# ishovkun/poroelasticity-dealii

Measured on AMD Instinct MI355X. Metric: DoF-updates/sec in assemble+SpMV per fixed-stress iter, higher is better.
Workload: dtype f64

## Files before the change

poroelasticity_dealii_amd/csrc/common.hpp:

```cpp
#pragma once
#include <hip/hip_runtime.h>
#include <cstdint>
#include <cstdio>
#include <map>
#include <memory>
#include <type_traits>
#include <stdexcept>
#include <string>
#include <list>
#include <vector>
#include "../../include/poroel_hip.h"
#include "fdm_tables.hpp"
#include "cell_field.hpp"

namespace poro {

#define PORO_HIP(x)                                                                                   \
  do { hipError_t e_ = (x); if (e_ != hipSuccess) throw poro::Error(std::string(#x) + " -> " + hipGetErrorString(e_)); } while (0)

template <class T> struct DevBuf {
  T *p = nullptr; size_t n = 0;
  DevBuf() = default; DevBuf(const DevBuf &) = delete; DevBuf &operator=(const DevBuf &) = delete;
  ~DevBuf() { release(); }
  void release() { if (p) (void)hipFree(p); p = nullptr; n = 0; }
  void alloc(size_t n_) { release(); n = n_; if (n) PORO_HIP(hipMalloc((void **)&p, n * sizeof(T))); }
  void zero(hipStream_t s) { if (n) PORO_HIP(hipMemsetAsync(p, 0, n * sizeof(T), s)); }
  void upload(const T *h, size_t n_) { alloc(n_); if (n) PORO_HIP(hipMemcpy(p, h, n * sizeof(T), hipMemcpyHostToDevice)); }
  void upload(const std::vector<T> &h) { upload(h.data(), h.size()); }
};

constexpr int kMaxPartials = 1024;
constexpr int kScalarSlots = 32;

struct PcgScalars {
  double dh, gg, gz;
  double gh2[2];
  double alpha, beta;
  double tol, res0, res;
  int32_t it, done, converged, max_iter, finishing;
  int32_t stop;
};
struct PcgStopTest { PcgScalars *sc = nullptr; const double *gg_part = nullptr; int it = 0; int per_wave = 0; };
static_assert(sizeof(PcgStopTest) == 24, "PcgStopTest is embedded in kernel arguments");

struct Mailbox { volatile unsigned long long seq; unsigned long long pad_; double vals[16]; PcgScalars sc; };

struct Cg1State { double gamma_old, alpha_old, alpha, beta, tol, res0, res; int32_t it, done, converged, pad_; };

struct DiagVec { const double *full = nullptr; const uint8_t *cls = nullptr; const double *tab = nullptr; int ncomp = 1; };

struct FeTablesDev {
  int nq_u, nq_p, nq_f, ns_u, ns_p;
  const double *w_qu, *w_qp, *w_qf, *u_qu, *du_qu, *du_qp, *q1_qu, *dq1_qu, *q1_qp, *dq1_qp, *u_qf, *dq1_qf;
};

struct BoxCoupling { int k; int n[3]; double h[3]; double N[3][2], D[3][2]; };

struct FdmDir { int n = 0; DevBuf<double> S, St, lam; };
struct FdmScalar { int dim = 0; FdmDir dir[3]; bool built = false; };
struct FdmScale { const double *lam[3]; int n[3]; double a, k[3]; int64_t ncol, col0, col_total; };
struct FdmWindow { int n_planes; int64_t ncols_valid, grid_col0, grid_plane0; };
struct SlabLayout {
  int n_ranks = 1, rank = 0;
  std::vector<int> layers, off;
  int ng = 0;
  int64_t ncol_total = 0, C = 0;
  int max_own = 0, max_nl = 0;
};
struct FdmDist : SlabLayout {
  bool built = false;
  FdmDir last;
  DevBuf<double> sendbuf, recvbuf, tz1, tz2; std::vector<double> hsend, hrecv;
  DevBuf<FdmWindow> windows;
};

struct FdmuDir { int n = 0; bool reg_form = false, split = false, blk = false; int n_even = 0; int blk_kk[2] = {0, 0}, blk_nch[2] = {0, 0}, blk_mb[2] = {0, 0} ; DevBuf<double> fwd, bwd, lam; };
struct FdmU : SlabLayout {
              int dim = 0; int nn[3] = {1, 1, 1}; double coef[3][3] = {}; FdmuDir dir[3][3]; FdmuDir last_global[3]; bool built = false, single = false;
              int fix[3][3][2] = {};
              bool dist = false; DevBuf<double> sendbuf, recvbuf, tz1, tz2;
              bool line = false; DevBuf<double> line_coef, line_fac; };
struct FdmoPlans;
constexpr double kFdmoStripFill = 0.4;
struct FdmOct {
  bool built = false; int nt = 0;
  int n[3] = {1, 1, 1}, h[3] = {1, 1, 1}; int hxp = 2;
  int64_t co_stride = 0, n_oct = 0;
  double coef[3][3] = {};
  DevBuf<double> fwd[3][3][2], bwd[3][3][2], lam[3][3][2];
  DevBuf<float> fwd32[3][3][2], bwd32[3][3][2];
  DevBuf<double> g, z, t;
  DevBuf<double> gz_part; int gz_n = 0;
  std::vector<double> h_lam[3][3][2];
  DevBuf<double> bxy;
  int no = 8;
  int nc = 3;
  bool planar = false;
  int own_z = 0;
  bool per_dir = false; int split_mask = 7, nt_z = 0;
  struct Slab {
    bool on = false; int n_ranks = 1, rank = 0;
    int ng = 0, hzg = 0;
    bool zboth = false; DevBuf<int64_t> dst2;
    int np = 2, nb = 12;
    int cw = 64, nchunk = 0, cps = 0, chunk0 = 0, my_chunks = 0;
    int64_t scols = 0;
    int own = 0, nl = 0, max_own = 0, max_nl = 0, rows_back = 0;
    int64_t recv_off = 0;
    DevBuf<int64_t> row_in;
    DevBuf<int64_t> row_out; DevBuf<int32_t> row_kz;
    DevBuf<double> buf, tz;
  } slab;
  std::shared_ptr<FdmoPlans> plans;
  struct ScalarTable { double a, kappa; DevBuf<double> t; };
  std::list<ScalarTable> scalar_tables;
  double strip_limit = 0;
};
struct FdmQ1 { FdmScalar nodal; FdmOct fused; };
struct SsorLevels { DevBuf<int32_t> fwd_rows, bwd_rows; std::vector<int64_t> fwd_off, bwd_off; bool built = false; };
struct CsrDev {
  int64_t n = 0, nnz = 0;
  DevBuf<int64_t> rp; DevBuf<int32_t> col; DevBuf<int64_t> diag_pos;
  int lanes_per_row = 8;
  SsorLevels ssor;
};

struct ConsDev {
  int64_t n = 0, n_masters = 0;
  DevBuf<int32_t> dof, master; DevBuf<int64_t> ptr; DevBuf<double> weight, inhom;
  DevBuf<int32_t> t_master, t_dof; DevBuf<int64_t> t_ptr; DevBuf<double> t_weight;
  DevBuf<uint8_t> inert;
  DevBuf<uint8_t> hanging;
  bool any_inhom = false;
};

struct Timer { double seconds = 0; int64_t launches = 0 , enqueued = 0 ; std::vector<std::pair<hipEvent_t, hipEvent_t>> pending;
               bool sample(int stride) { return enqueued++ % stride == 0; } };

struct IfcDev {
  int64_t m_send = 0, m_shared = 0, n_owned = 0;
  std::vector<int64_t> ptr;
  DevBuf<int32_t> dof, sh_dof, sh_src; DevBuf<int64_t> sh_ptr; DevBuf<double> send, recv;
  std::vector<double> hsend, hrecv;
};

struct Comm {
  poro_partition part{};
  bool general = false; std::vector<int32_t> neighbours; IfcDev ifc_u, ifc_p;
  void *nccl_comm = nullptr;
  poro_allreduce_fn ar = nullptr; poro_sendrecv_fn sr = nullptr; void *user = nullptr;
  DevBuf<double> recv_lo, recv_hi; std::vector<double> hsend, hrecv;
  struct Pinned { double *p = nullptr; size_t n = 0; Pinned() = default; Pinned(const Pinned &) = delete; Pinned &operator=(const Pinned &) = delete; ~Pinned() { if (p) (void)hipHostFree(p); } } hvec;
  bool force_multi = false;
  bool multi() const { return part.n_ranks > 1 || force_multi; }
};

struct KellyDev { bool built = false; int64_t n_faces = 0; DevBuf<int32_t> cell_a, cell_b, code, ent_face, ent_hcell; DevBuf<int64_t> ent_ptr; DevBuf<double> jump, eta; };

struct HybridPlan {
  bool built = false;
  int64_t n_box_nodes = 0, n_fine_cells = 0, n_removed = 0, n_chunks = 0;
  DevBuf<int64_t> inj;
  DevBuf<int32_t> color_cells; std::vector<int64_t> color_off;
  DevBuf<int32_t> spatial_cells;
  DevBuf<int32_t> removed_cells, slot;
  DevBuf<uint8_t> touched;
  DevBuf<double> Ke_t, V;
  DevBuf<int64_t> nodes; DevBuf<int32_t> chunk_cls;
  DevBuf<double> x_box, y_box;
};

struct BoxDev { int enabled = 0; int n[3] = {1, 1, 1}; int nn[3] = {1, 1, 1}; double h[3] = {1, 1, 1}; };

}

struct poro_ctx {
  poro_ctx() = default; poro_ctx(const poro_ctx &) = delete; poro_ctx &operator=(const poro_ctx &) = delete;
  ~poro_ctx() { if (mailbox) (void)hipHostFree(mailbox); }
  int device = 0, operator_mode = PORO_OP_CSR;
  hipStream_t stream = nullptr;
  int dim = 2, k_u = 2, ns_u = 9, ns_p = 4, dpc_u = 18, dpc_p = 4, nv = 4;
  int64_t n_cells = 0, n_u = 0, n_p = 0;
  poro_material mat{};
  poro::BoxDev box;
  struct Lines { bool on = false, uniform = true; int n[3] = {1, 1, 1}, nn[3] = {1, 1, 1}; std::vector<double> hcell[3]; } lines;
  poro::Comm comm;
  poro::DevBuf<int32_t> cell_dofs_u, cell_dofs_p, color_cells;
  poro::DevBuf<double> cell_X, tables;
  poro::DevBuf<double> cell_geo;
  poro::FeTablesDev fe{};
  int mfg_sf = 0;
  std::vector<int64_t> color_off;
  int scatter_mode = 0; poro::DevBuf<int32_t> spatial_cells;
  int operator_form = 0; poro::HybridPlan hyb;
  int fdm_precision = 0;
  int fdm_form = 0; bool fdm_form_fixed = false;
  poro::DevBuf<uint8_t> dir_mask, node_mask; poro::DevBuf<double> dir_val; poro::DevBuf<int32_t> dir_dofs;
  std::vector<int32_t> h_dir_dof; std::vector<double> h_dir_val;
  poro::ConsDev cons_u, cons_p;
  poro::DevBuf<uint8_t> pdir_mask; poro::DevBuf<double> pdir_val; int64_t n_pdir = 0;
  bool pdir_faces_ok = false; int pdir_face[3][2] = {{0, 0}, {0, 0}, {0, 0}};
  poro::DevBuf<int32_t> bface_cell, bface_local, bface_id, neu_label, neu_comp; poro::DevBuf<double> neu_val;
  poro::DevBuf<int32_t> bface_order; std::vector<int64_t> bface_group_off;
  int64_t n_bfaces = 0; int n_neumann = 0;
  poro::CsrDev Ap, Au;
  poro::DevBuf<double> Mp, Kp, Jp, Au_val;
  bool projection_matrix_ready = false;
  poro::DevBuf<double> Ke;
  std::map<int, poro::DevBuf<double>> vec, vec_saved;
  poro::DevBuf<uint8_t> rhs_u_flags;
  poro::DevBuf<double> lift_u, neumann_u, diag_u, diag_u_local, diag_J, diag_M, src_local;
  poro::DevBuf<double> dinv_u, dinv_J, dinv_M;
  poro::DevBuf<uint8_t> diag_u_cls; poro::DevBuf<double> diag_u_tab;
  poro::DevBuf<double> wg_u, wd_u, wh_u, wg_p, wd_p, wh_p, tmp_p, proj_y;
  bool box_asm_checked = false;
  int box_asm = 0 ; poro::BoxCoupling box_cpl{};
  poro::DevBuf<double> ilu_u, ilu_J, ilu_M; bool ilu_u_valid = false, ilu_J_valid = false, ilu_M_valid = false;
  poro::DevBuf<double> wz_p;
  poro::FdmQ1 q1_free, q1_fixed; poro::FdmDist fdm_dist; poro::DevBuf<double> fdm_t1, fdm_t2;
  double cheb_lmax = 0;
  double cheb_ratio_default = 0;
  poro::DevBuf<double> cheb_z, cheb_t;
  poro::FdmOct fdm_oct;
  struct Interp { int64_t n_fine = 0, n_coarse = 0; int lanes = 1, lanes_t = 1;    poro::DevBuf<int64_t> p_ptr, pt_ptr; poro::DevBuf<int32_t> p_col, pt_col; poro::DevBuf<double> p_w, pt_w; };
  struct TwoLevel : Interp { poro_ctx *box = nullptr; Interp pressure; bool pdir_nested = false;  } two_level;
  bool borrowed_stream = false;
  poro::FdmU fdm_u; poro::DevBuf<double> fdmu_t1, fdmu_t2, wz_u; int fdm_u_state = 0 ; std::string fdm_u_why;
  std::vector<uint8_t> h_node_mask;
  poro::DevBuf<double> partials; poro::DevBuf<poro::PcgScalars> scal; poro::DevBuf<double> red;
  poro::Mailbox *mailbox = nullptr; unsigned long long mb_seq = 0;
  int timing_stride = 1;
  poro::DevBuf<double> cheb_side_lo, cheb_side_hi;
  poro::DevBuf<poro::Cg1State> cg1_state; poro::DevBuf<double> cg1_z[2], cg1_w[2];
  bool matrix_built = false;
  int interleaved_u = 0;
  int pcg_hint_fdm_u[2] = {0, 0}, pcg_hint_cheb_u[2] = {0, 0}; int64_t cheb_applies = 0;
  int pcg_hint_u[2] = {0, 0};
  int pcg_hint_p[2] = {0, 0}, pcg_hint_proj[2] = {0, 0};
  int n_cus = 256; int mf_variant = 1 ; int mask_anywhere = 0;
  bool timing = false; std::map<std::string, poro::Timer> timers; std::vector<hipEvent_t> event_pool;
  double jac_dt = -1;
  poro::KellyDev kelly;
  struct Perm : poro::CellField<3> {
    int ncomp = 0;
    poro::DevBuf<double> cell, lattice;
    struct Line { bool built = false; int lo = 0, hi = 0; double a = -1; poro::DevBuf<double> coef, inv; } line[2];
  } perm;
  struct Moduli : poro::CellField<2> { poro::DevBuf<double> cell, node, planes; } mod;
  int moduli_op = 0;
  struct Gravity {
    bool on = false, loads_stale = false; double g[3] = {0, 0, 0}, rho_b = 0, rho_f = 0;
    struct Density : poro::CellField<1> { poro::DevBuf<double> cell, lattice; } dens;
    poro::DevBuf<double> body_u, flux_p, src_p;
    bool flux_on() const { return on && rho_f != 0; }
  } grav;
};

namespace poro {

inline bool box_fast_u(const poro_ctx *c) { return c->box.enabled && !c->mod.kind; }
inline bool moduli_structured_applies(const poro_ctx *c) {
  return c->box.enabled && c->dim == 3 && (c->k_u == 1 || c->k_u == 2) && c->mod.kind == 1 && c->operator_mode == PORO_OP_MATRIX_FREE && c->mf_variant == 1 && !c->comm.multi() &&
         c->comm.part.n_ranks <= 1;
}
inline bool moduli_structured(const poro_ctx *c) { return c->moduli_op == PORO_MODULI_OP_STRUCTURED && c->mod.planes.p && moduli_structured_applies(c); }

void la_fill(hipStream_t s, double *x, double v, int64_t n);
void la_nodal_interp(hipStream_t s, const int64_t *ptr, const int32_t *col, const double *w, int64_t n_rows, int ncomp, const double *in, double *out, int lanes = 1);
void la_two_level_combine(hipStream_t s, const int64_t *ptr, const int32_t *col, const double *w, int64_t n_rows, int ncomp, const double *zc, const double *g, const double *dinv, const uint8_t *inert, double omega, double *z, int lanes = 1);
void la_copy_many(hipStream_t s, int count, double *const *dst, const double *const *src, const int64_t *n);
void la_post(hipStream_t s, Mailbox *mb, unsigned long long seq, const double *src, int n, const PcgScalars *sc);
void la_reduce_post(hipStream_t s, const double *partials, int n_sets, double *red, int max_not_sum_mask, Mailbox *mb, unsigned long long seq);
void la_copy(hipStream_t s, double *y, const double *x, int64_t n);
void la_axpy(hipStream_t s, double *y, double a, const double *x, int64_t n);
void la_add_range(hipStream_t s, double *y, const double *x, int64_t n);
void la_add_two_ranges(hipStream_t s, double *y0, const double *x0, double *y1, const double *x1, int64_t n);
void la_dot_partials(hipStream_t s, const double *a, const double *b, int64_t n, double *partials , const PcgScalars *gate = nullptr );
void la_norm_partials(hipStream_t s, const double *a, int64_t n, double *partials_l2, double *partials_inf);
void la_reduce_finish(hipStream_t s, const double *partials, int n_sets, double *red , int max_not_sum_mask);
void la_csr_spmv(hipStream_t s, const CsrDev &A, const double *val, const double *x, double *y);
void la_csr_residual(hipStream_t s, const CsrDev &A, const double *M, const double *K, double kappa, const double *t, const double *p,
                     const double *src, double *R);
void la_pressure_tmp(hipStream_t s, double *t, const double *ev, const double *ev0, const double *p, const double *p_old, double c1, double c2, int64_t n);
void la_jacobian(hipStream_t s, double *J, const double *M, const double *K, double a, double kappa, int64_t nnz);
void la_ifc_pack(hipStream_t s, const IfcDev &I, const double *v);
void la_ifc_sum(hipStream_t s, const IfcDev &I, double *v);
void la_csr_diag(hipStream_t s, const CsrDev &A, const double *val, double *diag);
void la_reciprocal(hipStream_t s, double *y, const double *x, int64_t n);
void la_pointwise_mul(hipStream_t s, double *y, const double *x, int64_t n);
void la_cheb_first(hipStream_t s, double *z, const double *g, const DiagVec &dv, double scale, int64_t n);
void la_cheb_step(hipStream_t s, double *znew, const double *zj, const double *g, const double *Az, const DiagVec &dv, double omega, int64_t n, int64_t n_owned, double *gz_partials);
void la_cheb_fix_planes(hipStream_t s, double *znew, const double *zj, const double *g, const double *own_lo, const double *nbr_lo, const double *own_hi, const double *nbr_hi, const DiagVec &dv, double omega, int64_t n, int64_t plane);
void la_cons_expand(hipStream_t s, const ConsDev &C, double *x, bool with_inhom);
void la_cons_reduce(hipStream_t s, const ConsDev &C, double *y);
void la_xpby(hipStream_t s, double *y, double a, double b, const double *x, int64_t n);
void la_ilu0_factor(hipStream_t s, const CsrDev &A, const SsorLevels &lv, double *lu , int *flag );
void la_ilu_apply(hipStream_t s, const CsrDev &A, const double *lu, const SsorLevels &lv, const double *src, double *dst);
void la_ssor_apply(hipStream_t s, const CsrDev &A, const double *val, const SsorLevels &lv, double omega, const double *src, double *dst);
void la_sum_strains(hipStream_t s, double *ev, const double *const *strains, int n, int64_t len);
void la_effective_stress(hipStream_t s, const double *const *strains, double *const *stresses, int dim, double lam, double G, int64_t len);
void la_effective_stress_nodal(hipStream_t s, const double *const *strains, double *const *stresses, int dim, const double *node_mod, int64_t len);
void la_strain_update_nodal(hipStream_t s, double *ev, const double *dp, double alpha, const double *node_mod, int64_t len);
void la_set_constrained(hipStream_t s, double *x, const uint8_t *mask, const double *val, int64_t n);
void la_rhs_u_finish(hipStream_t s, double *rhs, const double *lift, const double *neumann, const uint8_t *mask, int64_t n);
void pcg_init_residual(hipStream_t s, double *g, const double *Ax, const double *b, const uint8_t *inert , int64_t n);
void la_mask_zero(hipStream_t s, double *x, const uint8_t *mask, int64_t n);
void pcg_dot_dh(hipStream_t s, const PcgScalars *sc, const double *d, const double *h, int64_t n_owned, double *partials);
void pcg_first_direction(hipStream_t s, double *d, const double *g, const DiagVec &diag, const double *z, int prec, int64_t n, int64_t n_owned, double *partials );
void pcg_scalars_sum(hipStream_t s, const double *partials, int n_sets, double *red);
void cg1_dots(hipStream_t s, const double *g, const double *z, const double *w, const double *b , int64_t n_owned, double *partials );
void cg1_scalars(hipStream_t s, Cg1State *st, const double *red, int first, double abs_tol, double rel_tol, int max_iter, int stop_rule);
void cg1_update(hipStream_t s, const Cg1State *st, double *d, double *sv, double *x, double *g, const double *z, const double *w, const DiagVec &dv, const uint8_t *inert,
                double *z1_out , double z1_scale, int64_t n);
void pcg_scalars_start(hipStream_t s, PcgScalars *sc, const double *red , double abs_tol, double rel_tol, int max_iter, int stop_rule);
void pcg_update_g_fused(hipStream_t s, PcgScalars *sc, int parity, double *g, const double *h, const DiagVec &diag, const double *z, double *z1_out , double z1_scale, int prec, int64_t n, int64_t n_owned,
                        const double *partials_dh, const double *red , double *partials_out );
void pcg_update_d_fused(hipStream_t s, PcgScalars *sc, int parity, int it, double *x, double *d, const double *g, const DiagVec &diag, const double *z, int prec, int64_t n,
                        const double *partials_in , const double *red );

void kelly_faces(hipStream_t s, int dim, int64_t n_faces, const int32_t *cell_a, const int32_t *cell_b, const int32_t *code, const double *cell_X, const int32_t *cell_dofs_p,
                 const double *p, double *jump);
void kelly_cells(hipStream_t s, int dim, int64_t n_cells, const int64_t *ent_ptr, const int32_t *ent_face, const int32_t *ent_hcell, const double *cell_X, const double *jump, double *eta);
void transfer_rows3(hipStream_t s, int64_t n_rows, const int64_t *ptr, const int32_t *col, const double *w, const double *const in[3], double *const out[3]);

struct AsmArgs {
  int dim, k_u, ns_u, ns_p, nv, dpc_u;
  FeTablesDev fe;
  const int32_t *cell_dofs_u, *cell_dofs_p; const double *cell_X;
  const double *cell_geo;
  const uint8_t *dir_mask; const double *dir_val;
  poro_material mat;
  int interleaved_u;
  int mfg_sf;
  const double *cell_mod;
};
void asm_u_matrix(hipStream_t s, const AsmArgs &a, const int32_t *cells, int64_t n_cells, const int64_t *rp, const int32_t *col, double *val, double *lift);
void asm_u_element_matrix(hipStream_t s, const AsmArgs &a, int32_t cell, double *Ke);
void asm_u_rhs(hipStream_t s, const AsmArgs &a, const int32_t *cells, int64_t n_cells, const double *p, double *rhs);
void asm_u_neumann(hipStream_t s, const AsmArgs &a, const int32_t *order, const std::vector<int64_t> &group_off, const int32_t *bf_cell, const int32_t *bf_local, const int32_t *bf_id,
                   int n_neu, const int32_t *label, const int32_t *comp, const double *value, double *rhs);
void asm_p_matrices(hipStream_t s, const AsmArgs &a, const int32_t *cells, int64_t n_cells, const int64_t *rp, const int32_t *col, double *M, double *K, double *src, const double *cell_w = nullptr,
                    int ncomp = 1);
void asm_proj_rhs(hipStream_t s, const AsmArgs &a, const int32_t *cells, int64_t n_cells, const double *u, int n_comp, const int32_t *comps ,
                  double *const *rhs );

void box_body_u(hipStream_t s, int dim, int k_u, const BoxDev &box, const double *rho_lattice, double rho0, const double *g, double *out);
void box_gravity_p(hipStream_t s, int dim, const BoxDev &box, const double *kap_lattice, int ncomp, double kap0, double rho_f, const double *g, double *out);
void asm_u_body(hipStream_t s, const AsmArgs &a, const int32_t *cells, int64_t n_cells, const double *cell_rho, double rho0, const double *g, double *out);
void asm_p_gravity(hipStream_t s, const AsmArgs &a, const int32_t *cells, int64_t n_cells, const double *cell_w, int ncomp, double kap0, double rho_f, const double *g, double *out);

bool mfg_sf_tables_match(const poro_fe_tables &f, int dim, int k);
int mfg_apply(hipStream_t s, const AsmArgs &a, const int32_t *color_cells, const std::vector<int64_t> &color_off, int64_t n_u, const double *x, double *y, bool constrained, int mode,
              const int32_t *all_cells = nullptr );
struct MfArgs { int dim, k_u; BoxDev box; const double *Ke; const uint8_t *mask; const double *diag_local; double lam, G; int mask_anywhere; const uint8_t *nodemask; const int32_t *dirichlet_dofs; int64_t n_dirichlet; };
void mf_apply(hipStream_t s, const MfArgs &a, const double *x, double *y, bool constrained, double *dot_partials = nullptr);
void mf_diag(hipStream_t s, const MfArgs &a, double *diag);
void p_stencil_apply(hipStream_t s, int dim, const BoxDev &box, double a, double kappa, const double *x, double *y);
void p_residual_stencil(hipStream_t s, int dim, const BoxDev &box, double kappa, const double *t, const double *p, const double *src, double *R);
void p_stencil_apply_var(hipStream_t s, int dim, const BoxDev &box, double a, const double *kap, int ncomp, const double *x, double *y);
void p_residual_stencil_var(hipStream_t s, int dim, const BoxDev &box, const double *kap, int ncomp, const double *t, const double *p, const double *src, double *R);

struct KronCheb { const double *g = nullptr; double *znew = nullptr; double omega = 0; const uint8_t *cls = nullptr; const double *tab = nullptr;
                  double *side_lo = nullptr, *side_hi = nullptr; };
bool kron_supported(int dim, int k_u);
void kron_prepare_device();
BoxCoupling box_coupling(int dim, int k_u, const BoxDev &box);
void box_rhs_u(hipStream_t s, int dim, const BoxCoupling &B, double alpha, const double *p, const double *lift, const double *neu, const uint8_t *mask, double *rhs,
               const uint8_t *flags = nullptr );
int64_t box_rhs_u_flag_count(int64_t n_u);
void box_rhs_u_flags(hipStream_t s, const double *lift, const double *neu, int64_t n_u, uint8_t *flags );
void box_asm_u_matrix(hipStream_t s, int dim, int k_u, const BoxDev &box, const double *Ke, const CsrDev &A, const uint8_t *mask, double *val);
void box_proj_rhs(hipStream_t s, int dim, const BoxCoupling &B, const double *u, int n_comp, const int32_t *tensor_components, double *const *rhs);
void fdm_window_batch(hipStream_t s, double *grid, double *dense, double *dense_self, int self, bool to_block, const FdmWindow *win, int n_peers, int n_planes_pad, int64_t C, int64_t grid_stride, int64_t blk);
void fdm_window(hipStream_t s, double *dst, const double *src, bool to_block, int n_planes, int n_planes_pad, int64_t C, int64_t ncols_valid, int64_t grid_stride, int64_t grid_col0, int64_t grid_plane0);
void fdm_transform(hipStream_t s, const double *T, int n_l, int64_t SI, int64_t n_outer, const double *in, double *out, const FdmScale *scale);
void q1_line_factor(hipStream_t s, int dim, int nw, const FdmScalar &F, int nl, double a, const double *coef, double *inv);
void q1_line_solve(hipStream_t s, int dim, int nw, const FdmScalar &F, int nl, double a, bool fixed_lo, bool fixed_hi, const double *coef, const double *inv, const double *in, double *out);
void fdm_apply(hipStream_t s, const FdmScalar &F, double a, const double k[3], const double *g, double *z, double *t1, double *t2);
void fdmu_upload_dir(FdmuDir &D, const LineTables &T, bool single, bool split);
void fdmu_apply(hipStream_t s, const FdmU &F, const double *g, double *z, void *t1, void *t2, int stage);
void fdmu_window(hipStream_t s, double *dst, const double *src, bool to_block, int ncomp, int n_planes, int n_planes_pad, int64_t C, int64_t ncols_valid,
                 int64_t grid_stride, int64_t grid_planes, int64_t grid_col0, int64_t grid_plane0);
void fdmu_lines(hipStream_t s, const FdmU &F, const FdmuDir *last_dir, int64_t C, int64_t col0, int64_t ncol_valid, void *in, void *out);
struct FdmuLineArgs { int nl, n0; int64_t ncol; const double *coef; const double *lam0[3], *lam1[3]; int fixed[3][2]; };
void fdmu_line_factor(hipStream_t s, int ku, int ncomp, const FdmuLineArgs &a, double *fac );
void fdmu_line_solve(hipStream_t s, int ku, int ncomp, const FdmuLineArgs &a, const double *fac, double *v );
bool fdmo_usable(int dim, const int nn[3]);
void fdmo_init(FdmOct &O, const int nn[3], const double coef[3][3], hipStream_t s);
void fdmo_init_slab(FdmOct &O, const int nn[3], const double coef[3][3], int rank, const std::vector<int> &node_layers, bool has_upper, hipStream_t s);
void fdmo_init_per_direction(FdmOct &O, const int nn[3], const double coef[3][3], const FdmFormDecision &D, hipStream_t s);
void fdmo_upload_dir(FdmOct &O, int comp, int dir, const LineTables &T);
void fdmo_finalize(FdmOct &O);
void fdmo_apply(hipStream_t s, const FdmOct &O, const double *g_oct, double *z_oct, double *scratch_oct, const PcgScalars *gate = nullptr, hipEvent_t *ev  = nullptr,
                double *gz_part  = nullptr,
                int precision  = PORO_FDM_FP64,
                const PcgStopTest &stop = PcgStopTest{} );
bool fdmo_scalar_usable(int dim, const int nn[3]);
void fdmo_scalar_init(FdmOct &O, const int nn[3], hipStream_t s);
void fdmo_scalar_upload_dir(FdmOct &O, int dir, const LineTables &T);
int fdmo_scalar_apply(hipStream_t s, FdmOct &O, double a, double kappa, const double *g, double *z, const PcgScalars *gate = nullptr);
int fdmo_scalar_apply_many(hipStream_t s, FdmOct &O, double a, double kappa, int nb, const double *const *g, double *const *z, const PcgScalars *gate = nullptr);
void la_residual_norms_many(hipStream_t s, int nb, const double *const *y, const double *const *b, int64_t n, double *partials, const uint8_t *mask = nullptr);
void fdmo_scalar_init_slab(FdmOct &O, const int nn[3], int rank, const std::vector<int> &node_layers, hipStream_t s);
void fdmo_scalar_slab_pass(hipStream_t s, FdmOct &O, int pass, double a, double kappa, const double *in, double *out);
bool fdmo_planar_usable(int dim, const int nn[3]);
void fdmo_init_planar(FdmOct &O, const int nn[3], const double coef[3][3], hipStream_t s, bool split = true );
void fdmo_upload_dir_planar(FdmOct &O, int comp, int dir, const LineTables &T);
void fdmo_apply_planar(hipStream_t s, const FdmOct &O, const double *g_q, double *z_q, const PcgScalars *gate = nullptr, const PcgStopTest &stop = PcgStopTest{} );
void fdmo_from_nodal(hipStream_t s, const FdmOct &O, const double *v_nodal, double *q_oct);
void fdmo_to_nodal(hipStream_t s, const FdmOct &O, const double *r_oct, double *v_nodal);
void fdmo_init_residual(hipStream_t s, const FdmOct &O, double *g_oct, const double *Ax, const double *b, const uint8_t *inert);
void fdmo_first_direction(hipStream_t s, const FdmOct &O, double *d, const double *g_oct, const double *z_oct, double *partials );
void fdmo_update_g(hipStream_t s, const FdmOct &O, PcgScalars *sc, int parity, double *g_oct, const double *h, const uint8_t *inert, const double *partials_dh, double *partials_out , const double *red = nullptr);
void fdmo_update_d(hipStream_t s, const FdmOct &O, PcgScalars *sc, int parity, int it, double *x, double *d, const double *z_oct, const double *partials_in , const double *red = nullptr,
                   bool gz_from_pass = false ,
                   bool stream_x = false ,
                   bool decided = false ,
                   bool gg_stored = false );
void fdmo_dot_owned(hipStream_t s, const FdmOct &O, const double *a_oct, const double *b_oct, double *partials, const PcgScalars *gate);
void fdmo_slab_pass(hipStream_t s, const FdmOct &O, int pass , const double *in, double *out, const PcgScalars *gate, hipEvent_t e0 = nullptr, hipEvent_t e1 = nullptr);
void fdmo_slab_scatter_pack(hipStream_t s, const FdmOct &O, const PcgScalars *gate);
int kron_apply(hipStream_t s, const MfArgs &a, const double *x, double *y, bool constrained, int n_cus, double *dot_partials = nullptr, hipEvent_t ev0 = nullptr, hipEvent_t ev1 = nullptr,
               const PcgScalars *pcg = nullptr ,
               const KronCheb *cheb = nullptr );
void kron_fix_constrained(hipStream_t s, const MfArgs &a, const double *x, double *y, double *dot_partials, int slot_base);
void kron_lm_prepare_device();
int kron_lm_apply(hipStream_t s, const MfArgs &a, const double *planes, const double *x, double *y, bool constrained, int n_cus, double *dot_partials = nullptr, hipEvent_t ev0 = nullptr,
                  hipEvent_t ev1 = nullptr, const PcgScalars *pcg = nullptr);
void hyb_gather(hipStream_t s, int dim, int64_t n_box_nodes, const int64_t *inj, const double *x, double *x_box);
struct HybCombine { int64_t n_box_nodes, n_removed, n_chunks; const int64_t *inj; const uint8_t *touched; const int32_t *removed_cells, *slot, *chunk_cls; const int64_t *nodes;
                    const double *x_box, *y_box; double *V; };
void hyb_combine(hipStream_t s, const MfArgs &box, const double *Ke_t, bool constrained, const HybCombine &h, double *y);

}
```

poroelasticity_dealii_amd/csrc/ctx_prec.hip:

```cpp
#include <dlfcn.h>
#include <rccl/rccl.h>
#include <algorithm>
#include <array>
#include <chrono>
#include <cmath>
#include <cstdlib>
#include <cstring>
#include <functional>
#include <new>
#include <optional>
#include <thread>
#include <unordered_map>
#include "common.hpp"
#include "ctx_internal.hpp"
#include "perm_line.hpp"
#include "moduli_line.hpp"

using namespace poro;
using namespace poro::ctx_detail;

namespace poro {
namespace ctx_detail {
bool fdm_p_supported(poro_ctx *c) {
  if (!c->lines.on) return false;
// ... 107 lines not shown
      PORO_HIP(hipMemcpyAsync(recv + (size_t)q * blk, F.hrecv.data(), blk * sizeof(double), hipMemcpyHostToDevice, c->stream)); PORO_HIP(hipStreamSynchronize(c->stream));
    }
  } else throw Error("partitioned context without a communicator");
}
void count_strip_launches(poro_ctx *c, int n) { if (n) c->timers["fdm_q1_strip_launches"].enqueued += n; }
void fdm_precondition_p(poro_ctx *c, double a, const double k[3], const double *g, double *z, Q1Set which) {
  Timed tm(c, "precondition_p_fdm");
  hipStream_t s = c->stream;
  const bool fixed = which == Q1Set::fixed_ends, isotropic = k[0] == k[1] && k[1] == k[2];
  FdmQ1 &T = q1_set(c, which);
  if (fixed || !c->comm.multi()) {
    std::optional<Timed> tf; if (fixed) tf.emplace(c, "precondition_p_fdm_fixed_ends");
    if (T.fused.built && isotropic) count_strip_launches(c, fdmo_scalar_apply(s, T.fused, a, k[0], g, z));
    else fdm_apply(s, T.nodal, a, k, g, z, c->fdm_t1.p, c->fdm_t2.p);
    return;
  }
  if (T.fused.built && T.fused.slab.on && isotropic) {
    FdmOct &O = T.fused; auto &S = O.slab; double *send = S.buf.p, *recv = S.buf.p + S.recv_off;
    fdmo_scalar_slab_pass(s, O, 1, a, k[0], g, S.buf.p);
    alltoall_blocks(c, send, recv, (int64_t)S.max_own * S.scols, true);
    fdmo_scalar_slab_pass(s, O, 2, a, k[0], S.buf.p, S.tz.p);
    fdmo_slab_scatter_pack(s, O, nullptr);
    alltoall_blocks(c, send, recv, (int64_t)S.max_nl * S.scols, true);
    fdmo_scalar_slab_pass(s, O, 3, a, k[0], S.buf.p, z);
    return;
  }
  FdmDist &F = c->fdm_dist; const FdmScalar &L = T.nodal;
  const int dim = c->dim, N = F.n_ranks, r = F.rank, last = dim - 1;
  const int n0 = L.dir[0].n, nl = c->box.n[last] + 1;
  const int64_t SIp = F.ncol_total;
  double *t1 = c->fdm_t1.p, *t2 = c->fdm_t2.p;
  const double *cur = g;
  if (dim == 3) { fdm_transform(s, L.dir[0].St.p, n0, 1, (int64_t)L.dir[1].n * nl, g, t1, nullptr); fdm_transform(s, L.dir[1].St.p, L.dir[1].n, n0, nl, t1, t2, nullptr); cur = t2; }
  else { fdm_transform(s, L.dir[0].St.p, n0, 1, nl, g, t1, nullptr); cur = t1; }
  const int64_t blk1 = (int64_t)F.max_own * F.C;
  fdm_window_batch(s, const_cast<double *>(cur), F.sendbuf.p, F.recvbuf.p, r, true, F.windows.p, N, F.max_own, F.C, SIp, blk1);
  alltoall_blocks(c, F.sendbuf.p, F.recvbuf.p, blk1, true);
  fdm_window_batch(s, F.tz1.p, F.recvbuf.p, nullptr, r, false, F.windows.p + N, N, F.max_own, F.C, F.C, blk1);
  FdmScale sc{}; sc.a = a; sc.ncol = F.C; sc.col0 = (int64_t)r * F.C; sc.col_total = F.ncol_total;
  for (int d = 0; d < 3; ++d) { sc.lam[d] = d < dim ? (d == last ? F.last.lam.p : L.dir[d].lam.p) : nullptr; sc.k[d] = d < dim ? k[d] : 0.0; sc.n[d] = d < dim ? (d == last ? F.ng : L.dir[d].n) : 1; }
  fdm_transform(s, F.last.St.p, F.ng, F.C, 1, F.tz1.p, F.tz2.p, &sc);
  fdm_transform(s, F.last.S.p, F.ng, F.C, 1, F.tz2.p, F.tz1.p, nullptr);
  const int64_t blk2 = (int64_t)F.max_nl * F.C;
  fdm_window_batch(s, F.tz1.p, F.sendbuf.p, F.recvbuf.p, r, true, F.windows.p + 2 * N, N, F.max_nl, F.C, F.C, blk2);
  alltoall_blocks(c, F.sendbuf.p, F.recvbuf.p, blk2, true);
  double *back = dim == 3 ? t2 : t1;
  fdm_window_batch(s, back, F.recvbuf.p, nullptr, r, false, F.windows.p + 3 * N, N, F.max_nl, F.C, SIp, blk2);
  if (dim == 3) { fdm_transform(s, L.dir[1].S.p, L.dir[1].n, n0, nl, t2, t1, nullptr); fdm_transform(s, L.dir[0].S.p, n0, 1, (int64_t)L.dir[1].n * nl, t1, z, nullptr); }
  else fdm_transform(s, L.dir[0].S.p, n0, 1, nl, t1, z, nullptr);
}

void fdm_precondition_p_layered(poro_ctx *c, double a, const double *g, double *z, Q1Set which) {
  Timed tm(c, "precondition_p_fdm_layered");
  const bool fixed = which == Q1Set::fixed_ends; const int last = c->dim - 1, nl = c->lines.n[last] + 1;
  poro_ctx::Perm &P = c->perm;
  if (!P.kind || c->comm.multi()) throw Error("fdm_precondition_p_layered: needs a per-cell permeability on a single-rank context");
  FdmQ1 &T = q1_set(c, which);
  const int nw = P.ncomp == 1 ? 1 : last;
  poro_ctx::Perm::Line &L = P.line[fixed ? 1 : 0];
  if (!L.built) {
    L.lo = fixed && c->pdir_face[last][0]; L.hi = fixed && c->pdir_face[last][1];
    L.coef.upload(perm_line_coefficients(c->lines.hcell[last], P.layer, nw, P.layer[P.ncomp - 1], L.lo, L.hi));
    if (L.inv.n != (size_t)c->n_p) L.inv.alloc(c->n_p);
    L.a = -1; L.built = true;
  }
  if (L.a != a) { q1_line_factor(c->stream, c->dim, nw, T.nodal, nl, a, L.coef.p, L.inv.p); L.a = a; }
  hipStream_t s = c->stream; const FdmScalar &F = T.nodal; const int n0 = F.dir[0].n, n1 = F.dir[1].n; double *t1 = c->fdm_t1.p, *t2 = c->fdm_t2.p;
  auto lines = [&](const double *in, double *out) { Timed tl(c, "q1_line_solve"); q1_line_solve(s, c->dim, nw, F, nl, a, L.lo, L.hi, L.coef.p, L.inv.p, in, out); };
  if (c->dim == 2) {
    fdm_transform(s, F.dir[0].St.p, n0, 1, nl, g, t1, nullptr);
    lines(t1, t2);
    fdm_transform(s, F.dir[0].S.p, n0, 1, nl, t2, z, nullptr);
  } else {
    fdm_transform(s, F.dir[0].St.p, n0, 1, (int64_t)n1 * nl, g, t1, nullptr);
    fdm_transform(s, F.dir[1].St.p, n1, n0, nl, t1, t2, nullptr);
    lines(t2, t1);
    fdm_transform(s, F.dir[1].S.p, n1, n0, nl, t1, t2, nullptr);
    fdm_transform(s, F.dir[0].S.p, n0, 1, (int64_t)n1 * nl, t2, z, nullptr);
  }
}

void analyse_fdm_u(poro_ctx *c) {
  if (c->fdm_u_state != 0) return;
  c->fdm_u_state = -1;
  const bool multi = c->comm.multi();
  if (multi && !(c->comm.nccl_comm || (c->comm.ar && c->comm.sr))) { c->fdm_u_state = 0; c->fdm_u_why = "partitioned context without a communicator yet"; return; }
  const int dim = c->dim, last = dim - 1; const int64_t nn[3] = {c->lines.nn[0], c->lines.nn[1], dim == 3 ? c->lines.nn[2] : 1};
  std::string why;
  FdmU &F = c->fdm_u;
  if (!c->lines.on || !c->interleaved_u || (multi && !c->box.enabled)) why = "needs a uniform box (or, on one rank, a tensor-product grid) with node-interleaved displacement dofs";
  else {
    for (int d = 0; d < dim; ++d) if (nn[d] > 4096) why = "more than 4096 nodes per grid line";
  }
  if (why.empty()) {
    const std::vector<uint8_t> &nm = c->h_node_mask;
    int physical[3][2] = {{1, 1}, {1, 1}, {1, 1}};
    if (multi) { physical[last][0] = !c->comm.part.has_lower; physical[last][1] = !c->comm.part.has_upper; }
    for (int comp = 0; comp < dim && why.empty(); ++comp)
      if (!whole_faces(nn, dim, nm.data(), comp, physical, F.fix[comp])) why = "Dirichlet dofs are not a union of whole faces per component";
  }
  if (multi) {
    double h[kScalarSlots] = {0}; int m = 0;
    for (int comp = 0; comp < 3; ++comp) for (int d = 0; d < 3; ++d) for (int side = 0; side < 2; ++side) h[m++] = (comp < dim && d < dim) ? F.fix[comp][d][side] : 0;
    h[m++] = why.empty() ? 0.0 : 1.0;
    PORO_HIP(hipMemcpyAsync(c->red.p, h, m * sizeof(double), hipMemcpyHostToDevice, c->stream));
    allreduce_sum(c, c->red.p, m);
    PORO_HIP(hipMemcpyAsync(h, c->red.p, m * sizeof(double), hipMemcpyDeviceToHost, c->stream)); PORO_HIP(hipStreamSynchronize(c->stream));
    m = 0;
    for (int comp = 0; comp < 3; ++comp) for (int d = 0; d < 3; ++d) for (int side = 0; side < 2; ++side) { if (comp < dim && d < dim) F.fix[comp][d][side] = h[m] > 0.5 ? 1 : 0; ++m; }
    if (h[m] > 0.5 && why.empty()) why = "another rank's Dirichlet dofs are not face-separable";
  }
  if (why.empty()) for (int d = 0; d < dim; ++d) {
    const int64_t line = (multi && d == last) ? 0 : nn[d];
    if (line > 320 && !(dim == 2 && !multi)) for (int comp = 0; comp < dim; ++comp) if (F.fix[comp][d][0] != F.fix[comp][d][1]) why = "a grid line of more than 320 points needs the same Dirichlet condition at both of its ends (even / odd transforms)";
  }
  if (why.empty()) for (int comp = 0; comp < dim; ++comp) {
    bool any = false;
    for (int d = 0; d < dim; ++d) any = any || F.fix[comp][d][0] || F.fix[comp][d][1];
    if (!any) why = "a displacement component without a constrained face (singular block)";
  }
  c->fdm_u_why = why;
  c->fdm_u_state = why.empty() ? 1 : -1;
}
void release_fdm_u(poro_ctx *c) {
  if (!c->fdm_u.built) return;
  PORO_HIP(hipStreamSynchronize(c->stream));
  c->fdm_oct.~FdmOct(); new (&c->fdm_oct) FdmOct();
  c->fdm_u.~FdmU(); new (&c->fdm_u) FdmU();
  c->fdm_u_state = 0; c->fdm_u_why.clear();
}
void build_fdm_u(poro_ctx *c) {
  FdmU &F = c->fdm_u;
  if (F.built) return;
  analyse_fdm_u(c);
  if (c->fdm_u_state != 1) throw Error("PORO_PREC_FDM (displacement): " + c->fdm_u_why);
  const int dim = c->dim, last = dim - 1, ku = c->k_u;
  const bool multi = c->comm.multi();
  const bool line = c->mod.kind != 0;
  if (line && multi) throw Error("PORO_PREC_FDM (displacement): per-cell moduli on a partitioned context");
  F.dim = dim; F.single = !multi && !line && std::getenv("PORO_FDMU_SINGLE") != nullptr;
  for (int d = 0; d < 3; ++d) F.nn[d] = d < dim ? c->lines.nn[d] : 1;
  const double l2g = c->mat.lame_lambda + 2 * c->mat.shear_G, G = c->mat.shear_G;
  for (int comp = 0; comp < dim; ++comp) for (int d = 0; d < dim; ++d) F.coef[comp][d] = d == comp ? l2g : G;
  int n_cells_last = c->lines.n[last];
  if (multi) {
    int64_t ncol_total = 1; for (int d = 0; d < last; ++d) ncol_total *= F.nn[d];
    F.dist = true; n_cells_last = slab_layout(c, F, ku, ncol_total);
    if (F.ng > 4096) throw Error("PORO_PREC_FDM (displacement): more than 4096 nodes per global grid line");
    const int N = F.n_ranks;
    const size_t blk = (size_t)dim * std::max(F.max_own, F.max_nl) * F.C;
    F.sendbuf.alloc(blk * N); F.recvbuf.alloc(blk * N); F.tz1.alloc((size_t)dim * F.ng * F.C); F.tz2.alloc((size_t)dim * F.ng * F.C);
    F.sendbuf.zero(c->stream); F.recvbuf.zero(c->stream); F.tz1.zero(c->stream); F.tz2.zero(c->stream);
  }
  LineTables tables[3][4]; bool same_ends[3], parity[3], parity_cd[3][3] = {};
  const auto key_of = [&](int comp, int d) { return F.fix[comp][d][0] * 2 + F.fix[comp][d][1]; };
  for (int d = 0; d < dim; ++d) {
    if (line && d == last) { same_ends[d] = parity[d] = false; continue; }
    const bool global_dir = multi && d == last;
    const std::vector<double> hcell = global_dir ? std::vector<double>((size_t)n_cells_last, c->box.h[d]) : c->lines.hcell[d];
    same_ends[d] = parity[d] = true;
    for (int comp = 0; comp < dim; ++comp) {
      LineTables &T = tables[d][key_of(comp, d)];
      if (!T.n) T = line_tables(ku, hcell, F.fix[comp][d][0], F.fix[comp][d][1]);
      same_ends[d] = same_ends[d] && F.fix[comp][d][0] == F.fix[comp][d][1]; parity[d] = parity[d] && T.parity; parity_cd[comp][d] = T.parity;
    }
  }
  bool oct_ok = !F.single && !line && !std::getenv("PORO_FDMU_NO_OCT");
  bool per_dir = false; FdmFormDecision form;
  bool planar = false;
  { int nn3[3] = {F.nn[0], F.nn[1], F.nn[2]}, sym3[3] = {F.nn[0], F.nn[1], multi ? F.ng : F.nn[2]};
    planar = dim == 2 && !multi && fdmo_planar_usable(dim, nn3);
    oct_ok = oct_ok && (planar || fdmo_usable(dim, sym3));
    bool symmetric = true, all_parity = true;
    for (int d = 0; d < dim; ++d) { symmetric = symmetric && same_ends[d]; all_parity = all_parity && parity[d]; }
    oct_ok = oct_ok && ((planar && !symmetric) || (symmetric && all_parity));
    if (c->fdm_form == PORO_FDM_FORM_PER_DIRECTION && !c->fdm_form_fixed && dim == 3 && !multi && !F.single && !line && !std::getenv("PORO_FDMU_NO_OCT")) {
      form = fdm_form_decide(F.fix, parity_cd, nn3);
      per_dir = form.usable && !form.all_split;
    }
    if (per_dir) { fdmo_init_per_direction(c->fdm_oct, nn3, F.coef, form, c->stream); oct_ok = true; }
    else if (oct_ok && planar) fdmo_init_planar(c->fdm_oct, nn3, F.coef, c->stream, symmetric);
    else if (oct_ok && !multi) fdmo_init(c->fdm_oct, nn3, F.coef, c->stream);
    if (oct_ok && multi) { std::vector<int> node_layers(F.n_ranks); for (int q = 0; q < F.n_ranks; ++q) node_layers[q] = ku * F.layers[q];
                           fdmo_init_slab(c->fdm_oct, nn3, F.coef, F.rank, node_layers, c->comm.part.has_upper != 0, c->stream); } }
  for (int d = 0; d < dim; ++d) for (int comp = 0; comp < dim; ++comp) {
    if (line && d == last) continue;
    const bool global_dir = multi && d == last;
    const LineTables &T = tables[d][key_of(comp, d)];
    FdmuDir &D = global_dir ? F.last_global[comp] : F.dir[comp][d];
    if (!(planar && oct_ok && T.n > 320 && !same_ends[d])) fdmu_upload_dir(D, T, global_dir ? false : F.single, same_ends[d] && parity[d]);
    if (oct_ok) { if (planar) fdmo_upload_dir_planar(c->fdm_oct, comp, d, T); else fdmo_upload_dir(c->fdm_oct, comp, d, T); }
  }
  c->fdmu_t1.alloc(c->n_u); c->fdmu_t2.alloc(c->n_u); c->fdmu_t1.zero(c->stream); c->fdmu_t2.zero(c->stream);
  if (!c->wz_u.p) { c->wz_u.alloc(c->n_u); c->wz_u.zero(c->stream); }
  if (oct_ok && !planar) fdmo_finalize(c->fdm_oct);
  c->fdm_oct.built = oct_ok;
  if (line) {
    std::vector<double> coef;
    for (int comp = 0; comp < dim; ++comp) {
      const std::vector<double> cc = moduli_line_coefficients(dim, ku, comp, c->lines.hcell[last], c->mod.layer[0], c->mod.layer[1], F.fix[comp][last][0] != 0, F.fix[comp][last][1] != 0);
      coef.insert(coef.end(), cc.begin(), cc.end());
    }
    F.line_coef.upload(coef);
    F.line_fac.alloc((size_t)(ku + 1) * c->n_u);
    F.line = true;
    fdmu_line_factor(c->stream, ku, dim, fdmu_line_args(c), F.line_fac.p);
  }
  F.built = true;
}
FdmuLineArgs fdmu_line_args(poro_ctx *c) {
  const FdmU &F = c->fdm_u; const int dim = F.dim, last = dim - 1;
  FdmuLineArgs a{};
  a.nl = F.nn[last]; a.n0 = F.nn[0]; a.ncol = c->n_u / dim / a.nl; a.coef = F.line_coef.p;
  for (int comp = 0; comp < dim; ++comp) {
    a.lam0[comp] = F.dir[comp][0].lam.p; a.lam1[comp] = dim == 3 ? F.dir[comp][1].lam.p : nullptr;
    a.fixed[comp][0] = F.fix[comp][last][0]; a.fixed[comp][1] = F.fix[comp][last][1];
  }
  return a;
}
static void fdm_precondition_u_slab(poro_ctx *c, const double *g, double *z, const PcgScalars *gate) {
  hipStream_t s = c->stream; FdmOct &O = c->fdm_oct; auto &S = O.slab;
  double *send = S.buf.p, *recv = S.buf.p + S.recv_off;
  fdmo_slab_pass(s, O, 1, g, S.buf.p, gate);
  alltoall_blocks(c, send, recv, (int64_t)S.max_own * S.scols, true);
  if (S.zboth) { Timed tp(c, "fdm_u_slab_z_stage"); fdmo_slab_pass(s, O, 2, S.buf.p, S.buf.p, gate); }
  else {
    fdmo_slab_pass(s, O, 2, S.buf.p, S.tz.p, gate);
    Timed tp(c, "fdm_u_slab_z_stage"); fdmo_slab_scatter_pack(s, O, gate);
  }
  alltoall_blocks(c, send, recv, (int64_t)S.max_nl * S.scols, true);
  fdmo_slab_pass(s, O, 3, S.buf.p, z, gate);
}
bool fdm_precondition_u_form(poro_ctx *c, const double *g, double *z, const PcgScalars *gate, int precision, double *scratch, double *gz_part, const PcgStopTest &stop) {
  Timed tm(c, "precondition_u_fdm");
  const FdmOct &O = c->fdm_oct;
  if (O.slab.on) { if (stop.gg_part) throw Error("fdm_precondition_u_form: the slab form runs no stopping test"); fdm_precondition_u_slab(c, g, z, gate); return false; }
  if (O.planar) { fdmo_apply_planar(c->stream, O, g, z, gate, stop); return false; }
  const char *names[3] = {"fdm_u_pass1", "fdm_u_pass2", "fdm_u_pass3"};
  if (!begin_sampled_dispatch(c, names[0])) {
    fdmo_apply(c->stream, O, g, z, scratch, gate, nullptr, gz_part, precision, stop);
    return gz_part != nullptr;
  }
  c->timers[names[1]].enqueued++;
  c->timers[names[2]].enqueued++;
  hipEvent_t ev[6];
  for (auto &e : ev) e = event_get(c);
  fdmo_apply(c->stream, O, g, z, scratch, gate, ev, gz_part, precision, stop);
  for (int k = 0; k < 3; ++k) {
    Timer &t = c->timers[names[k]];
    t.pending.emplace_back(ev[2 * k], ev[2 * k + 1]);
    t.launches++;
  }
  return gz_part != nullptr;
}
void fdm_precondition_u_nodal(poro_ctx *c, const double *g, double *z, int precision) {
  FdmOct &O = c->fdm_oct;
  if (!O.built) { fdm_precondition_u(c, g, z); return; }
  fdmo_from_nodal(c->stream, O, g, O.g.p); fdm_precondition_u_form(c, O.g.p, O.z.p, nullptr, precision, O.t.p); fdmo_to_nodal(c->stream, O, O.z.p, z);
}
static void upload_interp(poro_ctx::Interp &T, int64_t n_fine, int64_t n_owned, int64_t n_coarse, const int64_t *ptr, const int32_t *node, const double *weight, const char *what,
                          int row_bound = 0) {
  T.n_fine = n_fine; T.n_coarse = n_coarse;
  validate_rows(ptr, node, weight, n_fine, n_coarse, std::string("poro_desc.coarse: ") + what);
  const int64_t nnz = ptr[n_fine], nnz_t = ptr[n_owned];
  const auto lanes_for = [](int64_t nnz, int64_t rows) { return nnz >= 6 * rows ? 8 : nnz >= 3 * rows ? 4 : 1; };
  T.lanes = row_bound > 0 ? lanes_for(row_bound, 1) : lanes_for(nnz, n_fine); T.lanes_t = lanes_for(nnz_t, n_coarse);
  std::vector<int64_t> tp((size_t)n_coarse + 1, 0);
  for (int64_t k = 0; k < nnz_t; ++k) tp[node[k] + 1]++;
  { int64_t longest = 0; for (int64_t j = 0; j < n_coarse; ++j) longest = std::max(longest, tp[j + 1]);
    if (longest >= 48) T.lanes_t = std::max(T.lanes_t, 16); }
  for (int64_t j = 0; j < n_coarse; ++j) tp[j + 1] += tp[j];
  std::vector<int32_t> tc((size_t)nnz_t); std::vector<double> tw((size_t)nnz_t); std::vector<int64_t> pos(tp.begin(), tp.end() - 1);
  for (int64_t i = 0; i < n_fine; ++i) {
    if (i < n_owned) for (int64_t k = ptr[i]; k < ptr[i + 1]; ++k) { const int64_t at = pos[node[k]]++; tc[at] = (int32_t)i; tw[at] = weight[k]; }
  }
  T.p_ptr.upload(ptr, (size_t)n_fine + 1); T.p_col.upload(node, (size_t)nnz); T.p_w.upload(weight, (size_t)nnz);
  T.pt_ptr.upload(tp); T.pt_col.upload(tc); T.pt_w.upload(tw);
}
void setup_two_level(poro_ctx *c, const poro_desc *d) {
  auto &T = c->two_level; const int dim = c->dim;
  const bool general = c->comm.general;
  upload_interp(T, c->n_u / dim, general ? c->comm.ifc_u.n_owned / dim : c->n_u / dim, T.box->n_u / dim, d->coarse.ptr, d->coarse.node, d->coarse.weight, "displacement",
                general ? ipow(c->k_u + 1, dim) : 0);
  if (d->coarse.ptr_p) {
    if (!d->coarse.node_p || !d->coarse.weight_p) throw Error("poro_desc.coarse: node_p / weight_p missing");
    upload_interp(T.pressure, c->n_p, general ? c->comm.ifc_p.n_owned : c->n_p, T.box->n_p, d->coarse.ptr_p, d->coarse.node_p, d->coarse.weight_p, "pressure", general ? 1 << dim : 0);
    T.pdir_nested = false;
    const poro_desc *H = d->coarse.box_problem;
    if (c->n_pdir && H->n_dirichlet_p > 0 && H->dirichlet_dof_p) {
      std::vector<uint8_t> fine(c->n_p, 0), coarse(T.box->n_p, 0);
      for (int64_t i = 0; i < d->n_dirichlet_p; ++i) fine[d->dirichlet_dof_p[i]] = 1;
      for (int64_t i = 0; i < H->n_dirichlet_p; ++i) coarse[H->dirichlet_dof_p[i]] = 1;
      bool ok = true;
      for (int64_t i = 0; i < c->n_p && ok; ++i) {
        const int64_t k = d->coarse.ptr_p[i];
        if (d->coarse.ptr_p[i + 1] - k == 1 && std::fabs(d->coarse.weight_p[k] - 1.0) <= 1e-12 && coarse[d->coarse.node_p[k]] && !fine[i]) ok = false;
      }
      T.pdir_nested = ok;
    }
  }
}
bool two_level_supported(poro_ctx *c) {
  if (!c->two_level.box) return false;
  analyse_fdm_u(c->two_level.box);
  return c->two_level.box->fdm_u_state == 1;
}
bool two_level_supported_p(poro_ctx *c) { return c->two_level.box && c->two_level.pressure.n_fine == c->n_p && fdm_p_supported(c->two_level.box); }
bool two_level_supported_pj(poro_ctx *c) {
  return c->n_pdir && two_level_supported_p(c) && c->two_level.pdir_nested && c->two_level.box->n_pdir && fdm_pj_supported(c->two_level.box);
}
void two_level_precondition_p(poro_ctx *c, double a, double kappa, const double *dinv, const double *g, double *z, double omega, const uint8_t *inert, Q1Set coarse_set) {
  Timed tm(c, "precondition_p_two_level");
  auto &T = c->two_level.pressure; poro_ctx *H = c->two_level.box; hipStream_t s = c->stream;
  build_fdm_q1(H, coarse_set);
  if (!H->wz_p.p) H->wz_p.alloc(H->n_p);
  double *rc = H->wg_p.p, *zc = H->wz_p.p;
  la_nodal_interp(s, T.pt_ptr.p, T.pt_col.p, T.pt_w.p, T.n_coarse, 1, g, rc, T.lanes_t);
  if (c->comm.multi()) allreduce_sum_vec(c, rc, T.n_coarse, "two_level_coarse_allreduce");
  const double kk[3] = {kappa, kappa, kappa};
  fdm_precondition_p(H, a, kk, rc, zc, coarse_set);
  la_two_level_combine(s, T.p_ptr.p, T.p_col.p, T.p_w.p, T.n_fine, 1, zc, g, dinv, inert, omega, z, T.lanes);
}
void two_level_precondition_u(poro_ctx *c, const double *g, double *z, double omega) {
  Timed tm(c, "precondition_u_two_level");
  auto &T = c->two_level; poro_ctx *H = T.box; hipStream_t s = c->stream; const int dim = c->dim;
  build_fdm_u(H);
  double *rc = H->wg_u.p, *zc = H->wz_u.p;
  la_nodal_interp(s, T.pt_ptr.p, T.pt_col.p, T.pt_w.p, T.n_coarse, dim, g, rc, T.lanes_t);
  if (c->comm.multi()) allreduce_sum_vec(c, rc, T.n_coarse * dim, "two_level_coarse_allreduce");
  fdm_precondition_u_nodal(H, rc, zc, PORO_FDM_FP64);
  la_two_level_combine(s, T.p_ptr.p, T.p_col.p, T.p_w.p, T.n_fine, dim, zc, g, c->dinv_u.p, c->cons_u.inert.p, omega, z, T.lanes);
}

void fdm_precondition_u(poro_ctx *c, const double *g, double *z) {
  Timed tm(c, "precondition_u_fdm");
  hipStream_t s = c->stream; FdmU &F = c->fdm_u;
  if (F.line) {
    fdmu_apply(s, F, g, z, c->fdmu_t1.p, c->fdmu_t2.p, 0);
    { Timed tl(c, "fdm_u_line_solve"); fdmu_line_solve(s, c->k_u, F.dim, fdmu_line_args(c), F.line_fac.p, F.dim == 3 ? c->fdmu_t2.p : c->fdmu_t1.p); }
    fdmu_apply(s, F, g, z, c->fdmu_t1.p, c->fdmu_t2.p, 1);
    return;
  }
  if (!F.dist) { fdmu_apply(s, F, g, z, c->fdmu_t1.p, c->fdmu_t2.p, 2); return; }
  const int dim = F.dim, N = F.n_ranks, r = F.rank, last = dim - 1, ku = c->k_u;
  const int nl = F.nn[last];
  fdmu_apply(s, F, g, z, c->fdmu_t1.p, c->fdmu_t2.p, 0);
  double *cur = dim == 3 ? c->fdmu_t2.p : c->fdmu_t1.p;
  auto ncols_of = [&](int q) { return std::max<int64_t>(0, std::min<int64_t>(F.C, F.ncol_total - (int64_t)q * F.C)); };
  auto own_of = [&](int q) { return ku * F.layers[q] + (q == N - 1 ? 1 : 0); };
  const int64_t blk1 = (int64_t)dim * F.max_own * F.C;
  for (int q = 0; q < N; ++q) fdmu_window(s, F.sendbuf.p + (size_t)q * blk1, cur, true, dim, own_of(r), F.max_own, F.C, ncols_of(q), F.ncol_total, nl, (int64_t)q * F.C, 0);
  alltoall_blocks(c, F.sendbuf.p, F.recvbuf.p, blk1);
  PORO_HIP(hipMemsetAsync(F.tz1.p, 0, (size_t)dim * F.ng * F.C * sizeof(double), s));
  for (int q = 0; q < N; ++q) fdmu_window(s, F.tz1.p, F.recvbuf.p + (size_t)q * blk1, false, dim, own_of(q), F.max_own, F.C, F.C, F.C, F.ng, 0, F.off[q]);
  fdmu_lines(s, F, F.last_global, F.C, (int64_t)r * F.C, ncols_of(r), F.tz1.p, F.tz2.p);
  const int64_t blk2 = (int64_t)dim * F.max_nl * F.C;
  for (int q = 0; q < N; ++q) fdmu_window(s, F.sendbuf.p + (size_t)q * blk2, F.tz2.p, true, dim, ku * F.layers[q] + 1, F.max_nl, F.C, F.C, F.C, F.ng, 0, F.off[q]);
  alltoall_blocks(c, F.sendbuf.p, F.recvbuf.p, blk2);
  for (int q = 0; q < N; ++q) fdmu_window(s, cur, F.recvbuf.p + (size_t)q * blk2, false, dim, nl, F.max_nl, F.C, ncols_of(q), F.ncol_total, nl, (int64_t)q * F.C, 0);
  fdmu_apply(s, F, g, z, c->fdmu_t1.p, c->fdmu_t2.p, 1);
}

const char *prec_refusal(poro_ctx *c, int which_system, int prec, bool solving) {
  static thread_local std::string why;
  if (prec == PORO_PREC_NONE || prec == PORO_PREC_JACOBI) return nullptr;
  const bool multi = c->comm.multi(), sweeps = prec == PORO_PREC_SSOR || prec == PORO_PREC_ILU0;
  const char *one_rank = prec == PORO_PREC_SSOR ? "PORO_PREC_SSOR is a single-rank fidelity mode (the sweeps are order dependent)"
                                                : "PORO_PREC_ILU0 is implemented for one rank (the factorisation is sequential in the row order)";
  if (which_system == 0) {
    if (c->mod.kind && prec == PORO_PREC_TWO_LEVEL)
      return "PORO_PREC_TWO_LEVEL (displacement): not available while per-cell moduli are set - the coarse box is a constant-coefficient context (PORO_PREC_JACOBI / CHEBYSHEV / NONE everywhere, ILU0 / SSOR on the assembled operator, PORO_PREC_FDM on boxes and tensor-product grids)";
    if (prec == PORO_PREC_TWO_LEVEL)
      return two_level_supported(c) ? nullptr : "PORO_PREC_TWO_LEVEL needs poro_desc.coarse (a refinement of a uniform box whose Dirichlet conditions cover whole faces)";
    if (c->cons_u.n && prec != PORO_PREC_CHEBYSHEV) return "meshes with constraint lists: PORO_PREC_JACOBI / CHEBYSHEV / TWO_LEVEL / NONE only (the operator is condensed on the fly)";
    if (prec == PORO_PREC_CHEBYSHEV) return nullptr;
    if (sweeps) return c->operator_mode != PORO_OP_CSR ? (prec == PORO_PREC_SSOR ? "PORO_PREC_SSOR needs the assembled CSR operator" : "PORO_PREC_ILU0 needs the assembled CSR operator") : multi ? one_rank : nullptr;
    if (prec == PORO_PREC_FDM) {
      analyse_fdm_u(c);
      if (c->fdm_u_state == 1) return nullptr;
      why = "PORO_PREC_FDM (displacement): " + c->fdm_u_why;
      return why.c_str();
    }
    return solving ? nullptr : "unknown preconditioner";
  }
  if (which_system != 1 && which_system != 2) return "unknown system (0 displacement, 1 pressure, 2 projection)";
  if (which_system == 1 && c->perm.kind && prec == PORO_PREC_TWO_LEVEL)
    return "PORO_PREC_TWO_LEVEL (pressure): not available while a per-cell permeability is set - the coarse box is a constant-coefficient context (PORO_PREC_JACOBI / NONE / ILU0 / SSOR everywhere, PORO_PREC_FDM on boxes and tensor-product grids)";
  if (which_system == 1 && (c->cons_p.n || c->n_pdir)) {
    const bool ok = prec == PORO_PREC_TWO_LEVEL ? (!c->n_pdir || two_level_supported_pj(c)) : prec == PORO_PREC_FDM && fdm_pj_supported(c);
    if (!ok) return "meshes with hanging-node constraints or prescribed pressures: PORO_PREC_JACOBI / NONE (hanging nodes: also TWO_LEVEL; with prescribed pressures where the coarse box carries them as whole faces) only; prescribed pressures that cover whole faces of a uniform box or tensor-product grid on one rank: also PORO_PREC_FDM";
  }
// ... 11 lines not shown
```

poroelasticity_dealii_amd/csrc/fdm_tables.hpp:

```cpp
#pragma once
#include <algorithm>
#include <cmath>
#include <cstddef>
#include <limits>
#include <stdexcept>
#include <vector>

namespace poro {
struct Error : std::runtime_error { using std::runtime_error::runtime_error; };

inline void jacobi_eig(int n, std::vector<double> &A, std::vector<double> &V, std::vector<double> &w) {
  V.assign((size_t)n * n, 0.0); for (int i = 0; i < n; ++i) V[(size_t)i * n + i] = 1.0;
  for (int sweep = 0; sweep < 60; ++sweep) {
    double off = 0, diag = 0;
    for (int i = 0; i < n; ++i) { diag += A[(size_t)i * n + i] * A[(size_t)i * n + i]; for (int j = i + 1; j < n; ++j) off += A[(size_t)i * n + j] * A[(size_t)i * n + j]; }
    if (off <= 1e-30 * diag || off == 0) break;
    for (int p = 0; p < n - 1; ++p)
      for (int q = p + 1; q < n; ++q) {
        const double apq = A[(size_t)p * n + q];
        if (std::fabs(apq) < 1e-300) continue;
        const double app = A[(size_t)p * n + p], aqq = A[(size_t)q * n + q];
        const double theta = (aqq - app) / (2.0 * apq);
        const double t = (theta >= 0 ? 1.0 : -1.0) / (std::fabs(theta) + std::sqrt(theta * theta + 1.0));
        const double cs = 1.0 / std::sqrt(t * t + 1.0), sn = t * cs;
// ... 68 lines not shown
        for (i = m - 1; i >= l; --i) {
          double f = sn * e[i]; const double b = cs * e[i];
          e[i + 1] = (r = std::hypot(f, g));
          if (r == 0.0) { d[i + 1] -= p; e[m] = 0.0; break; }
          sn = f / r; cs = g / r; g = d[i + 1] - p;
          r = (d[i] - g) * sn + 2.0 * cs * b;
          d[i + 1] = g + (p = sn * r); g = cs * r - b;
          for (int k = 0; k < n; ++k) { f = a(k, i + 1); a(k, i + 1) = sn * a(k, i) + cs * f; a(k, i) = cs * a(k, i) - sn * f; }
        }
        if (r == 0.0 && i >= l) continue;
        d[l] -= p; e[l] = g; e[m] = 0.0;
      }
    } while (m != l);
  }
  V = A; w = d;
}

inline double sym_lambda_max(int n, const std::vector<double> &A) {
  std::vector<double> B = A, V, w; jacobi_eig(n, B, V, w);
  double m = 0; for (double v : w) m = std::max(m, v);
  return m;
}
inline double jacobi_scaled_lambda_max(int n, const std::vector<double> &A) {
  std::vector<double> B((size_t)n * n), V, w;
  for (int i = 0; i < n; ++i) for (int j = 0; j < n; ++j) B[(size_t)i * n + j] = 0.5 * (A[(size_t)i * n + j] + A[(size_t)j * n + i]) / std::sqrt(A[(size_t)i * n + i] * A[(size_t)j * n + j]);
  jacobi_eig(n, B, V, w);
  double m = 0; for (double v : w) m = std::max(m, v);
  return m;
}

struct LineTables { int n = 0; std::vector<double> S, lam; bool parity = false; std::vector<int> even, odd; };
inline void classify_parity(LineTables &T) {
  const int n = T.n, h = (n + 1) / 2; const std::vector<double> &S = T.S;
  T.parity = true; T.even.clear(); T.odd.clear();
  for (int m = 0; m < n && T.parity; ++m) {
    if (!(T.lam[m] < 1e300)) continue;
    double ds = 0, da = 0, nrm = 0;
    for (int k = 0; k < n; ++k) { const double a = S[(size_t)k * n + m], b = S[(size_t)(n - 1 - k) * n + m]; ds += (a - b) * (a - b); da += (a + b) * (a + b); nrm += a * a; }
    if (ds <= 1e-20 * nrm) T.even.push_back(m); else if (da <= 1e-20 * nrm) T.odd.push_back(m); else T.parity = false;
  }
  T.parity = T.parity && (int)T.even.size() <= h && (int)T.odd.size() <= h;
  if (!T.parity) { T.even.clear(); T.odd.clear(); }
}
inline void fe1d(int k, const std::vector<double> &hc, std::vector<double> &M, std::vector<double> &K) {
  const int n_cells = (int)hc.size(), nn = k * n_cells + 1; M.assign((size_t)nn * nn, 0.0); K.assign((size_t)nn * nn, 0.0);
  static const double M2[3][3] = {{4, 2, -1}, {2, 16, 2}, {-1, 2, 4}}, K2[3][3] = {{7, -8, 1}, {-8, 16, -8}, {1, -8, 7}};
  static const double M1[2][2] = {{2, 1}, {1, 2}}, K1[2][2] = {{1, -1}, {-1, 1}};
  for (int c = 0; c < n_cells; ++c)
    for (int a = 0; a <= k; ++a) for (int b = 0; b <= k; ++b) {
      const size_t at = (size_t)(k * c + a) * nn + (k * c + b);
      const double h = hc[c];
      if (k == 2) { M[at] += h / 30.0 * M2[a][b]; K[at] += K2[a][b] / (3.0 * h); } else { M[at] += h / 6.0 * M1[a][b]; K[at] += K1[a][b] / h; }
    }
}

inline LineTables line_tables(int k, const std::vector<double> &hc, bool fix_lo, bool fix_hi) {
  const int n_cells = (int)hc.size();
  std::vector<double> M, K; fe1d(k, hc, M, K);
  const int nn = k * n_cells + 1, f0 = fix_lo ? 1 : 0, nf = nn - f0 - (fix_hi ? 1 : 0);
  LineTables T; T.n = nn; std::vector<double> &S = T.S, &lam = T.lam;
  S.assign((size_t)nn * nn, 0.0); lam.assign(nn, std::numeric_limits<double>::infinity());
  if (nf <= 0) return T;
  std::vector<double> Lc((size_t)nf * nf, 0.0), C((size_t)nf * nf);
  for (int i = 0; i < nf; ++i)
    for (int j = 0; j <= i; ++j) {
      double s = M[(size_t)(i + f0) * nn + (j + f0)];
      for (int p = 0; p < j; ++p) s -= Lc[(size_t)i * nf + p] * Lc[(size_t)j * nf + p];
      if (i == j) { if (!(s > 0)) throw Error("fdmu_eig_1d: mass matrix not positive definite"); Lc[(size_t)i * nf + i] = std::sqrt(s); }
      else Lc[(size_t)i * nf + j] = s / Lc[(size_t)j * nf + j];
    }
  std::vector<double> X((size_t)nf * nf);
  for (int col = 0; col < nf; ++col)
    for (int i = 0; i < nf; ++i) {
      double s = K[(size_t)(i + f0) * nn + (col + f0)];
      for (int p = 0; p < i; ++p) s -= Lc[(size_t)i * nf + p] * X[(size_t)p * nf + col];
      X[(size_t)i * nf + col] = s / Lc[(size_t)i * nf + i];
    }
  for (int row = 0; row < nf; ++row)
    for (int i = 0; i < nf; ++i) {
      double s = X[(size_t)row * nf + i];
      for (int p = 0; p < i; ++p) s -= Lc[(size_t)i * nf + p] * C[(size_t)p * nf + row];
      C[(size_t)i * nf + row] = s / Lc[(size_t)i * nf + i];
    }
  for (int i = 0; i < nf; ++i) for (int j = i + 1; j < nf; ++j) { const double a = 0.5 * (C[(size_t)i * nf + j] + C[(size_t)j * nf + i]); C[(size_t)i * nf + j] = C[(size_t)j * nf + i] = a; }
  std::vector<double> Q, wv;
  if (nf > 96) householder_ql_eig(nf, C, Q, wv); else jacobi_eig(nf, C, Q, wv);
  for (int j = 0; j < nf; ++j) {
    std::vector<double> sv(nf);
    for (int i = nf - 1; i >= 0; --i) {
      double s = Q[(size_t)i * nf + j];
      for (int p = i + 1; p < nf; ++p) s -= Lc[(size_t)p * nf + i] * sv[p];
      sv[i] = s / Lc[(size_t)i * nf + i];
    }
    for (int i = 0; i < nf; ++i) S[(size_t)(i + f0) * nn + j] = sv[i];
    lam[j] = std::max(wv[j], 0.0);
  }
  if (fix_lo == fix_hi)
    for (int j = 0; j < nf; ++j) {
      double ds = 0, da = 0;
      for (int k = 0; k < nn; ++k) { const double a = S[(size_t)k * nn + j], b = S[(size_t)(nn - 1 - k) * nn + j]; ds += (a - b) * (a - b); da += (a + b) * (a + b); }
      const double sgn = ds <= da ? 1.0 : -1.0;
      if (std::min(ds, da) > 1e-8 * std::max(ds, da)) continue;
      for (int k = 0; k < nn / 2; ++k) {
        const double a = S[(size_t)k * nn + j], b = S[(size_t)(nn - 1 - k) * nn + j], v = 0.5 * (a + sgn * b);
        S[(size_t)k * nn + j] = v; S[(size_t)(nn - 1 - k) * nn + j] = sgn * v;
      }
      if ((nn & 1) && sgn < 0) S[(size_t)(nn / 2) * nn + j] = 0.0;
      double nrm = 0;
      for (int i = 0; i < nn; ++i) { double t = 0; for (int p = std::max(0, i - 2 * k); p <= std::min(nn - 1, i + 2 * k); ++p) t += M[(size_t)i * nn + p] * S[(size_t)p * nn + j]; nrm += S[(size_t)i * nn + j] * t; }
      const double sc = 1.0 / std::sqrt(nrm);
      for (int i = 0; i < nn; ++i) S[(size_t)i * nn + j] *= sc;
    }
  classify_parity(T);
  return T;
}

inline LineTables q1_eig(int n_cells, double h) {
  const int n = n_cells + 1; const double pi = 3.14159265358979323846;
  LineTables T; T.n = n; std::vector<double> &S = T.S, &lam = T.lam;
  S.assign((size_t)n * n, 0.0); lam.assign(n, 0.0);
  std::vector<double> v(n);
  for (int j = 0; j < n; ++j) {
    const double t = j * pi / n_cells, ct = std::cos(t);
    lam[j] = 6.0 / (h * h) * (1.0 - ct) / (2.0 + ct);
    for (int i = 0; i < n; ++i) v[i] = std::cos(t * i);
    double m = 0;
    for (int i = 0; i < n; ++i) {
      double Mv = (i > 0 && i < n - 1 ? 4.0 : 2.0) * v[i];
      if (i > 0) Mv += v[i - 1];
      if (i < n - 1) Mv += v[i + 1];
      m += v[i] * Mv * h / 6.0;
    }
    const double sc = 1.0 / std::sqrt(m);
    for (int i = 0; i < n; ++i) S[(size_t)i * n + j] = v[i] * sc;
  }
  classify_parity(T);
  return T;
}

template <class T, class El> std::vector<T> pack_fragments(int tiles, int ksteps, int rows, int cols, El el) {
  std::vector<T> f((size_t)tiles * ksteps * 64, (T)0);
  for (int t = 0; t < tiles; ++t) for (int kk = 0; kk < ksteps; ++kk) for (int l = 0; l < 64; ++l) {
    const int r = 16 * t + (l & 15), c = 4 * kk + (l >> 4);
    if (r < rows && c < cols) f[((size_t)t * ksteps + kk) * 64 + l] = (T)el(r, c);
  }
  return f;
}
inline std::vector<double> whole_line_fragments(const LineTables &T, int tiles, bool backward) {
  const int n = T.n; const std::vector<double> &S = T.S;
  return backward ? pack_fragments<double>(tiles, 4 * tiles, n, n, [&](int r, int c) { return S[(size_t)r * n + c]; })
                  : pack_fragments<double>(tiles, 4 * tiles, n, n, [&](int r, int c) { return S[(size_t)c * n + r]; });
}

constexpr int kFdmoMaxTiles = 8;
struct FdmFormDecision { bool usable = false, all_split = false; int split[3] = {0, 0, 0}, len[3] = {0, 0, 0}; int nt_xy = 0, nt_z = 0, parts = 1; };
inline FdmFormDecision fdm_form_decide(const int fix[3][3][2], const bool parity[3][3] , const int nn[3]) {
  FdmFormDecision D; D.usable = true; D.all_split = true;
  for (int d = 0; d < 3; ++d) {
    bool split = true;
    for (int c = 0; c < 3; ++c) split = split && fix[c][d][0] == fix[c][d][1] && parity[c][d];
    D.split[d] = split ? 1 : 0; D.len[d] = split ? (nn[d] + 1) / 2 : nn[d];
    D.all_split = D.all_split && split; if (split) D.parts *= 2;
    if (nn[d] < 2 || D.len[d] > 16 * kFdmoMaxTiles) D.usable = false;
  }
  D.nt_xy = (std::max(D.len[0], D.len[1]) + 15) / 16; D.nt_z = (D.len[2] + 15) / 16;
  return D;
}

template <class Tile, class El> std::vector<double> pack_paired_chunks(int blocks, int chunks, int pairs, Tile tile, El el) {
  std::vector<double> f((size_t)blocks * chunks * 4 * pairs * 128, 0.0);
  for (int b = 0; b < blocks; ++b) for (int ch = 0; ch < chunks; ++ch) for (int u = 0; u < 4; ++u) for (int p = 0; p < pairs; ++p) for (int l = 0; l < 64; ++l) for (int e = 0; e < 2; ++e) {
    const int r = 16 * tile(b, p, e) + (l & 15), c = 4 * (4 * ch + u) + (l >> 4);
    f[((((size_t)(b * chunks + ch) * 4 + u) * pairs + p) * 64 + l) * 2 + e] = el(r, c, e);
  }
  return f;
}

}
```

poroelasticity_dealii_amd/csrc/kernels_fdmo.hip:

```cpp
#include "common.hpp"
#include "fdm_tables.hpp"
#include "device_reduce.hpp"
#include <hip/hip_ext.h>
#include <cmath>
#include <cstdlib>
#include <limits>
#include <mutex>
#include <set>
#include <type_traits>

namespace poro {
namespace {

typedef double v4d __attribute__((ext_vector_type(4)));
typedef float v4f __attribute__((ext_vector_type(4)));

struct OctDims { int nx, ny, nz, hx, hy, hz, hxp; int64_t co; int no, own_z, nc; int split; int part[8]; };

__device__ __forceinline__ void bfly_fwd(double (&v)[8], const bool (&centre)[3]) {
#pragma unroll
  for (int bit = 0; bit < 3; ++bit) {
    const int m = 1 << bit;
#pragma unroll
    for (int i = 0; i < 8; ++i) if (!(i & m)) {
// ... 284 lines not shown
  const double *__restrict__ T1 = static_cast<const double *>(P.T1[c][(o >> P.bit1) & 1]) + lane, *__restrict__ T2 = static_cast<const double *>(P.T2[c][(o >> P.bit2) & 1]) + lane;
  int slab_q0 = 0, slab_sw = 0; int64_t slab_base[2] = {0, 0};
  if (MODE != 1 && f_slab_io) {
    const int X0 = co * P.col_unit; slab_q0 = X0 / P.scols; slab_sw = (slab_q0 + 1) * P.scols - X0;
    for (int k = 0; k < 2; ++k) slab_base[k] = (int64_t)X0 + (int64_t)(slab_q0 + k) * P.dest_stride + (int64_t)b * P.scols + ((f_slab_io == 2 || slab_q0 + k == P.rank) ? P.recv_off : 0);
  }
  auto slab_at = [&](int col) -> int64_t {
    if (P.scols >= P.col_unit) return (int64_t)col + (col >= slab_sw ? slab_base[1] : slab_base[0]);
    const int X = co * P.col_unit + col;
    int q = (int)((float)X * P.inv_scols); q -= q * P.scols > X; q += (q + 1) * P.scols <= X;
    return (int64_t)X + (int64_t)q * P.dest_stride + (int64_t)b * P.scols + ((f_slab_io == 2 || q == P.rank) ? P.recv_off : 0);
  };
  auto stamp = [&](int k) { if (P.stamps && tid == 0) P.stamps[(int64_t)blockIdx.x * 8 + k] = __builtin_amdgcn_s_memrealtime(); };
  stamp(0);
  {
    constexpr int HP = PADC / 2, TOT = Gm::PADN * HP, PER = (TOT + 64 * NW - 1) / (64 * NW);
    double2 stage[PER];
#pragma unroll
    for (int u = 0; u < PER; ++u) {
      const int e = tid + u * 64 * NW, r = e / HP, c2 = 2 * (e - r * HP);
      if (MODE == 1 && f_row_in) {
        const bool ok = e < TOT && r < R && c2 < C, split = f_slab_z == 2; const int rr = ok ? r : 0, mr = split ? P.ng - 1 - rr : rr; const int64_t cb = (int64_t)(blockIdx.x >> (f_slab_z - 1)) * P.C + c2;
        const double2 lo = ok ? *reinterpret_cast<const double2 *>(in + f_row_in[rr] + cb) : double2{0.0, 0.0}, hi = (ok && mr != rr) ? *reinterpret_cast<const double2 *>(in + f_row_in[mr] + cb) : double2{0.0, 0.0};
        const bool odd = split && (blockIdx.x & 1);
        stage[u].x = odd ? (mr != rr ? lo.x - hi.x : 0.0) : lo.x + hi.x; stage[u].y = odd ? (mr != rr ? lo.y - hi.y : 0.0) : lo.y + hi.y;
      } else if (MODE == 2 && f_slab_io == 2) {
        if (f_vec2) stage[u] = (e < TOT && r < R && c2 < C) ? *reinterpret_cast<const double2 *>(in + slab_at(r * (int)P.row_stride + c2)) : double2{0.0, 0.0};
        else { stage[u].x = (e < TOT && r < R && c2 < C) ? in[slab_at(r * (int)P.row_stride + c2)] : 0.0; stage[u].y = (e < TOT && r < R && c2 + 1 < C) ? in[slab_at(r * (int)P.row_stride + c2 + 1)] : 0.0; }
      }
      else if (f_vec2) stage[u] = (e < TOT && r < R && c2 < C) ? *reinterpret_cast<const double2 *>(in + base_in + (int64_t)r * P.row_stride + c2) : double2{0.0, 0.0};
      else { const double *src = in + base_in + (int64_t)r * P.row_stride + c2; stage[u].x = (e < TOT && r < R && c2 < C) ? src[0] : 0.0; stage[u].y = (e < TOT && r < R && c2 + 1 < C) ? src[1] : 0.0; }
    }
    if constexpr (QUARTERS) { if (stop_pending) pcg_stop_post_quarter(stop_q, stop_wave); }
#pragma unroll
    for (int u = 0; u < PER; ++u) { const int e = tid + u * 64 * NW, r = e / HP, c2 = 2 * (e - r * HP); if (e < TOT) *reinterpret_cast<double2 *>(&L[r * LD1 + c2]) = stage[u]; }
  }
  constexpr int CHK = EXTRA ? 2 : 4, NCH = Gm::KKP / CHK;
  double tf[2][NS][CHK];
  auto load_chunk = [&](int buf, int step) {
    const double *__restrict__ T = step < NCH ? T1 : T2; const int ch = step < NCH ? step : step - NCH;
#pragma unroll
    for (int k = 0; k < CHK; ++k) {
      tf[buf][0][k] = T[((int64_t)w * Gm::KKP + CHK * ch + k) * 64];
      if constexpr (EXTRA) tf[buf][1][k] = T[((int64_t)XT * Gm::KKP + CHK * ch + k) * 64];
    }
  };
  v4d acc[NACC];
  auto zero_acc = [&]() {
#pragma unroll
    for (int t = 0; t < NACC; ++t) acc[t] = v4d{0, 0, 0, 0};
  };
  auto gemm = [&](auto contract_cols, auto ld_c, auto first_step_c, auto corner_c, int kk_n) {
    constexpr bool kCols = decltype(contract_cols)::value, kCorner = decltype(corner_c)::value; constexpr int LD = decltype(ld_c)::value, S0 = decltype(first_step_c)::value;
    const double *La = kCols ? L + j * LD + kq : L + kq * LD + j;
    const double *Lw = kCols ? La + 16 * w * LD : La + 16 * w;
#pragma unroll
    for (int ch = 0; ch < NCH; ++ch) {
      const int buf = (S0 + ch) & 1;
#pragma unroll
      for (int k = 0; k < CHK; ++k) {
        const int kk = CHK * ch + k;
        if (kk < Gm::KKP - 3 || kk < kk_n) {
          double d[NT];
#pragma unroll
          for (int t = 0; t < NT; ++t) if (t < NL || (kCorner && t == XT)) d[t] = kCols ? La[16 * t * LD + 4 * kk] : La[4 * kk * LD + 16 * t];
          double dw = 0; if constexpr (EXTRA) dw = kCols ? Lw[4 * kk] : Lw[4 * kk * LD];
#pragma unroll
          for (int t = 0; t < NL; ++t) acc[t] = kCols ? __builtin_amdgcn_mfma_f64_16x16x4f64(d[t], tf[buf][0][k], acc[t], 0, 0, 0) : __builtin_amdgcn_mfma_f64_16x16x4f64(tf[buf][0][k], d[t], acc[t], 0, 0, 0);
          if constexpr (EXTRA) acc[NL] = kCols ? __builtin_amdgcn_mfma_f64_16x16x4f64(dw, tf[buf][1][k], acc[NL], 0, 0, 0) : __builtin_amdgcn_mfma_f64_16x16x4f64(tf[buf][1][k], dw, acc[NL], 0, 0, 0);
          if constexpr (kCorner) acc[NL + 1] = kCols ? __builtin_amdgcn_mfma_f64_16x16x4f64(d[XT], tf[buf][1][k], acc[NL + 1], 0, 0, 0) : __builtin_amdgcn_mfma_f64_16x16x4f64(tf[buf][1][k], d[XT], acc[NL + 1], 0, 0, 0);
        }
      }
      if (S0 + ch + 2 < 2 * NCH) load_chunk(buf, S0 + ch + 2);
    }
  };
  auto tile_of = [&](int a, int &tr, int &tc, bool cols) {
    if (a < NL) { tr = cols ? a : w; tc = cols ? w : a; }
    else if (a == NL) { tr = cols ? w : XT; tc = cols ? XT : w; }
    else { tr = XT; tc = XT; }
  };
  typedef std::integral_constant<bool, kColsFirst> CF; typedef std::integral_constant<int, LD1> L1c;
  typedef std::integral_constant<bool, kColsSecond> CS; typedef std::integral_constant<int, LD2> L2c;
  typedef std::integral_constant<int, 0> S0c; typedef std::integral_constant<int, NCH> S1c;
  __builtin_amdgcn_s_setprio(3);
  load_chunk(0, 0); load_chunk(1, 1);
  zero_acc();
  __builtin_amdgcn_s_setprio(0);
  __syncthreads();
  if constexpr (QUARTERS) { if (stop_pending && pcg_stop_decide_quarters(P.stop, stop_q, stop_wave)) return; }
  stamp(1);
  if (heavy) gemm(CF{}, L1c{}, S0c{}, std::integral_constant<bool, CORNER>{}, P.kk1); else gemm(CF{}, L1c{}, S0c{}, std::false_type{}, P.kk1);
  __syncthreads();
  stamp(2);
  if constexpr (MODE == 1) {
    const double *lamz = P.lam_z[c][(o >> (PERDIR ? P.bitz : 2)) & 1], *bx = P.bxy + (int64_t)(f_bxy_cmul * c + (PERDIR ? (o & (P.bxy_cmul - 1)) : (o & 3))) * P.pl;
    const double czc = P.cz[c];
    double lzw[4], lzx[4];
#pragma unroll
    for (int q = 0; q < 4; ++q) { lzw[q] = czc * lamz[16 * w + 4 * q + kq]; lzx[q] = EXTRA ? czc * lamz[16 * XT + 4 * q + kq] : 0.0; }
    double gz = 0;
#pragma unroll
    for (int a = 0; a < NACC; ++a) {
      int tr, tc; tile_of(a, tr, tc, false);
      const double bxy = bx[min(b * P.C + 16 * tc + j, P.pl - 1)];
#pragma unroll
      for (int q = 0; q < 4; ++q) {
        const double den = (a < NL ? lzw[q] : lzx[q]) + bxy;
        double r = __builtin_amdgcn_rcp(den);
        r = den < 1e300 ? fma(r, fma(-den, r, 1.0), r) : 0.0;
        const double zh = acc[a][q] * r;
        L[(16 * tr + 4 * q + kq) * LD2 + 16 * tc + j] = zh;
        if constexpr (GZ) gz = fma(acc[a][q], zh, gz);
        __builtin_amdgcn_sched_barrier(0);
      }
    }
    if constexpr (GZ) {
      gz = wave_sum(gz);
      if (lane == 0) gz_wave[w] = gz;
    }
  } else {
#pragma unroll
    for (int a = 0; a < NACC; ++a) {
      int tr, tc; tile_of(a, tr, tc, kColsFirst);
      if (a == NL + 1 && !heavy) continue;
#pragma unroll
      for (int q = 0; q < 4; ++q) L[(16 * tr + 4 * q + kq) * LD2 + 16 * tc + j] = acc[a][q];
    }
  }
  zero_acc();
  __syncthreads();
  stamp(3);
  if constexpr (GZ) {
    if (tid == 0) { double t = 0; for (int k = 0; k < NW; ++k) t += gz_wave[k]; P.gz_part[blockIdx.x] = t; }
  }
  if (heavy) gemm(CS{}, L2c{}, S1c{}, std::integral_constant<bool, CORNER>{}, P.kk2); else gemm(CS{}, L2c{}, S1c{}, std::false_type{}, P.kk2);
  if (P.stamps) { __syncthreads(); stamp(4); }
#pragma unroll
  for (int a = 0; a < NACC; ++a) {
    int tr, tc; tile_of(a, tr, tc, kColsSecond);
    if (a == NL + 1 && !heavy) continue;
#pragma unroll
    for (int q = 0; q < 4; ++q) {
      const int r = 16 * tr + 4 * q + kq, cc = 16 * tc + j;
      if (MODE == 0 && f_slab_io == 1) { if (r < R && cc < C && b < P.store_planes) out[slab_at(r * (int)P.row_stride + cc)] = acc[a][q]; }
      else if (r < R && cc < C) out[base_out + (int64_t)r * P.row_stride + cc] = acc[a][q];
    }
  }
  if (P.stamps) {
    __builtin_amdgcn_s_waitcnt(0); __syncthreads(); stamp(5);
    if (tid == 0) { unsigned hw, xcc; asm volatile("s_getreg_b32 %0, hwreg(HW_REG_HW_ID)" : "=s"(hw)); asm volatile("s_getreg_b32 %0, hwreg(HW_REG_XCC_ID)" : "=s"(xcc)); P.stamps[(int64_t)blockIdx.x * 8 + 6] = hw; P.stamps[(int64_t)blockIdx.x * 8 + 7] = xcc; }
  }
}

template <int NT, int MODE>
__global__ void __launch_bounds__(64 * NT)
k_fdmo_strip(OctPass P, const double *in, double *out) {
  typedef PassGeom<NT> Gm;
  constexpr bool kColsFirst = MODE == 0, kColsSecond = MODE == 2;
  constexpr int LD1 = MODE == 1 ? 16 : (kColsFirst ? Gm::LDA : Gm::LDB), LD2 = MODE == 1 ? 16 : (kColsSecond ? Gm::LDA : Gm::LDB);
  constexpr int PADC = MODE == 1 ? 16 : Gm::PADN, KKP = Gm::KKP;
  extern __shared__ double L[];
  if (pcg_gate_closed(P.gate)) return;
  const int tid = threadIdx.x, lane = tid & 63, w = __builtin_amdgcn_readfirstlane(tid >> 6);
  const int j = lane & 15, kq = lane >> 4;
  const int item = MODE == 1 ? (int)blockIdx.x : (int)blockIdx.x / NT, s = MODE == 1 ? 0 : (int)blockIdx.x - item * NT;
  const int co = item / P.nblk, b = item - co * P.nblk;
  const int R = P.R, C = MODE == 1 ? min(P.C, P.pl - b * P.C) : P.C;
  if ((MODE == 0 && 16 * s >= C) || (MODE == 2 && 16 * s >= R)) return;
  const int64_t base = (int64_t)co * P.co_stride + (int64_t)b * P.blk_stride;
  const int64_t base_in = P.use_in_off ? (int64_t)b * P.blk_stride : base, base_out = P.use_out_off ? (int64_t)b * P.blk_stride : base;
  if (P.use_in_off) in = P.in_blk[co];
  if (P.use_out_off) out = P.out_blk[co];
  const int f1 = MODE == 1 ? w : s;
  const double *__restrict__ T1 = static_cast<const double *>(P.T1[co][0]) + (int64_t)f1 * KKP * 64 + lane, *__restrict__ T2 = static_cast<const double *>(P.T2[co][0]) + (int64_t)w * KKP * 64 + lane;
  double t1[KKP], t2[KKP];
#pragma unroll
  for (int kk = 0; kk < KKP; ++kk) t1[kk] = T1[kk * 64];
  {
    constexpr int TOT = Gm::PADN * PADC, PER = TOT / (64 * NT);
    static_assert(TOT % (64 * NT) == 0, "staging loop");
    double stage[PER];
#pragma unroll
    for (int u = 0; u < PER; ++u) { const int e = tid + u * 64 * NT, r = e / PADC, cc = e - r * PADC; stage[u] = (r < R && cc < C) ? in[base_in + (int64_t)r * P.row_stride + cc] : 0.0; }
#pragma unroll
    for (int u = 0; u < PER; ++u) { const int e = tid + u * 64 * NT, r = e / PADC, cc = e - r * PADC; L[r * LD1 + cc] = stage[u]; }
  }
#pragma unroll
  for (int kk = 0; kk < KKP; ++kk) t2[kk] = T2[kk * 64];
  __syncthreads();
  v4d acc = v4d{0, 0, 0, 0};
  {
    const double *La = kColsFirst ? L + (16 * w + j) * LD1 + kq : L + kq * LD1 + (MODE == 1 ? 0 : 16 * w) + j;
#pragma unroll
    for (int kk = 0; kk < KKP; ++kk) {
      if (kk < KKP - 3 || kk < P.kk1) {
        const double d = kColsFirst ? La[4 * kk] : La[4 * kk * LD1];
        acc = kColsFirst ? __builtin_amdgcn_mfma_f64_16x16x4f64(d, t1[kk], acc, 0, 0, 0) : __builtin_amdgcn_mfma_f64_16x16x4f64(t1[kk], d, acc, 0, 0, 0);
      }
    }
  }
  __syncthreads();
  {
    const int tr = MODE == 2 ? s : w, tc = MODE == 0 ? s : (MODE == 2 ? w : 0);
    if constexpr (MODE == 1) {
      const double *lamz = P.lam_z[co][0]; const double czc = P.cz[co];
      const double bxy = P.bxy[min(b * P.C + j, P.pl - 1)];
#pragma unroll
      for (int q = 0; q < 4; ++q) {
        const double den = fma(czc, lamz[16 * w + 4 * q + kq], bxy);
        double r = __builtin_amdgcn_rcp(den);
        r = den < 1e300 ? fma(r, fma(-den, r, 1.0), r) : 0.0;
        L[(16 * tr + 4 * q + kq) * LD2 + 16 * tc + j] = acc[q] * r;
      }
    } else {
#pragma unroll
      for (int q = 0; q < 4; ++q) L[(16 * tr + 4 * q + kq) * LD2 + 16 * tc + j] = acc[q];
    }
  }
  acc = v4d{0, 0, 0, 0};
  __syncthreads();
  {
    const double *La = kColsSecond ? L + (16 * s + j) * LD2 + kq : L + kq * LD2 + 16 * s + j;
#pragma unroll
    for (int kk = 0; kk < KKP; ++kk) {
      if (kk < KKP - 3 || kk < P.kk2) {
        const double d = kColsSecond ? La[4 * kk] : La[4 * kk * LD2];
        acc = kColsSecond ? __builtin_amdgcn_mfma_f64_16x16x4f64(d, t2[kk], acc, 0, 0, 0) : __builtin_amdgcn_mfma_f64_16x16x4f64(t2[kk], d, acc, 0, 0, 0);
      }
    }
  }
  {
    const int tr = MODE == 2 ? s : w, tc = MODE == 0 ? s : (MODE == 2 ? w : 0);
#pragma unroll
    for (int q = 0; q < 4; ++q) {
      const int r = 16 * tr + 4 * q + kq, cc = 16 * tc + j;
      if (r < R && cc < C) out[base_out + (int64_t)r * P.row_stride + cc] = acc[q];
    }
  }
}


template <int NT, int MODE, bool GZ = false>
__global__ void __launch_bounds__(64 * pass_waves<NT>())
k_fdmo_pass_f32(OctPass P, const double *in, double *out) {
  static_assert(!GZ || MODE == 1, "g . z comes out of pass 2");
  typedef PassGeom<NT> Gm;
  constexpr int NW = pass_waves<NT>();
  constexpr bool EXTRA = NT > NW;
  constexpr int XT = NT - 1;
  constexpr int NL = (MODE == 1 && EXTRA) ? NW : NT;
  constexpr bool CORNER = EXTRA && MODE != 1;
  constexpr int NACC = NL + (EXTRA ? 1 : 0) + (CORNER ? 1 : 0);
  constexpr bool kColsFirst = MODE == 0, kColsSecond = MODE == 2;
  constexpr int LD1 = kColsFirst ? Gm::LDA : Gm::LDB, LD2 = kColsSecond ? Gm::LDA : Gm::LDB;
  constexpr int NS = EXTRA ? 2 : 1;
  constexpr int PADC = 16 * NL;
  extern __shared__ float Lf[];
  __shared__ double gz_wave[GZ ? NW : 1];
  constexpr bool QUARTERS = MODE == 0 && NW == 4;
  __shared__ double stop_wave[QUARTERS ? 4 : 1];
  [[maybe_unused]] PcgStopQuarter stop_q; [[maybe_unused]] bool stop_pending = false;
  if (MODE == 0 && P.stop.gg_part) {
    if (QUARTERS && !P.stop.per_wave) {
      if (P.gate && (P.gate->done | P.gate->finishing)) return;
      pcg_stop_load_quarter(P.stop, stop_q); stop_pending = true;
    } else {
      PcgStopInputs stop_in;
      pcg_stop_load(P.stop, stop_in);
      if (P.gate && (P.gate->done | P.gate->finishing)) return;
      if (pcg_stop_decide(P.stop, stop_in)) return;
    }
  } else if (pcg_gate_closed(P.gate)) return;
  const int tid = threadIdx.x, lane = tid & 63, w = __builtin_amdgcn_readfirstlane(tid >> 6);
  const int j = lane & 15, kq = lane >> 4;
  auto arow = [&](int q) { return 4 * kq + q; };
  const int co = blockIdx.x / P.nblk, b = blockIdx.x % P.nblk, c = co >> 3, o = co & 7;
  const int64_t base = (int64_t)co * P.co_stride + (int64_t)b * P.blk_stride;
  const bool heavy = CORNER && w == (int)(blockIdx.x & (NW - 1));
  const int R = P.R, C = MODE == 1 ? min(P.C, P.pl - b * P.C) : P.C;
  const float *__restrict__ T1 = static_cast<const float *>(P.T1[c][(o >> P.bit1) & 1]) + lane, *__restrict__ T2 = static_cast<const float *>(P.T2[c][(o >> P.bit2) & 1]) + lane;
  const float *inf = reinterpret_cast<const float *>(in); float *outf = reinterpret_cast<float *>(out);
  {
    constexpr int HP = PADC / 2, TOT = Gm::PADN * HP, PER = (TOT + 64 * NW - 1) / (64 * NW);
    float2 stage[PER];
#pragma unroll
    for (int u = 0; u < PER; ++u) {
      const int e = tid + u * 64 * NW, r = e / HP, c2 = 2 * (e - r * HP);
      const bool ok = e < TOT && r < R && c2 < C; const int64_t at = base + (int64_t)r * P.row_stride + c2;
      if constexpr (MODE == 0) { const double2 v = ok ? *reinterpret_cast<const double2 *>(in + at) : double2{0.0, 0.0}; stage[u] = float2{(float)v.x, (float)v.y}; }
      else stage[u] = ok ? *reinterpret_cast<const float2 *>(inf + at) : float2{0.f, 0.f};
    }
    if constexpr (QUARTERS) { if (stop_pending) pcg_stop_post_quarter(stop_q, stop_wave); }
#pragma unroll
    for (int u = 0; u < PER; ++u) { const int e = tid + u * 64 * NW, r = e / HP, c2 = 2 * (e - r * HP); if (e < TOT) *reinterpret_cast<float2 *>(&Lf[r * LD1 + c2]) = stage[u]; }
  }
  constexpr int CHK = EXTRA ? 2 : 4, NCH = Gm::KKP / CHK;
  float tf[2][NS][CHK];
  auto load_chunk = [&](int buf, int step) {
    const float *__restrict__ T = step < NCH ? T1 : T2; const int ch = step < NCH ? step : step - NCH;
#pragma unroll
    for (int k = 0; k < CHK; ++k) {
      tf[buf][0][k] = T[((int64_t)w * Gm::KKP + CHK * ch + k) * 64];
      if constexpr (EXTRA) tf[buf][1][k] = T[((int64_t)XT * Gm::KKP + CHK * ch + k) * 64];
    }
  };
  v4f acc[NACC];
// ... 216 lines not shown
  double tf[2][NS][CHK];
  const double *__restrict__ T1e = static_cast<const double *>(P.T1[c][0]) + lane, *__restrict__ T1o = static_cast<const double *>(P.T1[c][1]) + lane, *__restrict__ T2e = static_cast<const double *>(P.T2[c][0]) + lane, *__restrict__ T2o = static_cast<const double *>(P.T2[c][1]) + lane;
  auto load_chunk = [&](int buf, int step) {
    const bool first = step < NCH; const int ch = first ? step : step - NCH;
    const double *__restrict__ Te = first ? T1e : T2e, *__restrict__ To = first ? T1o : T2o;
#pragma unroll
    for (int k = 0; k < CHK; ++k) {
      tf[buf][0][k] = Te[((int64_t)w * Gm::KKP + CHK * ch + k) * 64];
      tf[buf][1][k] = To[((int64_t)w * Gm::KKP + CHK * ch + k) * 64];
      if constexpr (EXTRA) tf[buf][2][k] = (pw ? To : Te)[((int64_t)XT * Gm::KKP + CHK * ch + k) * 64];
    }
  };
  v4d acc[NACC];
  auto zero_acc = [&]() {
#pragma unroll
    for (int t = 0; t < NACC; ++t) acc[t] = v4d{0, 0, 0, 0};
  };
  auto gemm = [&](auto first_step_c, int kk_n) {
    constexpr int S0 = decltype(first_step_c)::value;
    const double *La = L + kq * LD + j, *Lw = La + 16 * w;
#pragma unroll
    for (int ch = 0; ch < NCH; ++ch) {
      const int buf = (S0 + ch) & 1;
#pragma unroll
      for (int k = 0; k < CHK; ++k) {
        const int kk = CHK * ch + k;
        if (kk < Gm::KKP - 3 || kk < kk_n) {
          double d[NL];
#pragma unroll
          for (int t = 0; t < NL; ++t) d[t] = La[4 * kk * LD + 16 * t];
          double dw = 0; if constexpr (EXTRA) dw = Lw[4 * kk * LD];
#pragma unroll
          for (int t = 0; t < NL; ++t) acc[t] = __builtin_amdgcn_mfma_f64_16x16x4f64(tf[buf][t < HT ? 0 : 1][k], d[t], acc[t], 0, 0, 0);
          if constexpr (EXTRA) acc[NL] = __builtin_amdgcn_mfma_f64_16x16x4f64(tf[buf][2][k], dw, acc[NL], 0, 0, 0);
        }
      }
      if (S0 + ch + 2 < 2 * NCH) load_chunk(buf, S0 + ch + 2);
    }
  };
  __builtin_amdgcn_s_setprio(3);
  load_chunk(0, 0); load_chunk(1, 1);
  zero_acc();
  __builtin_amdgcn_s_setprio(0);
  __syncthreads();
  gemm(std::integral_constant<int, 0>{}, P.kk1);
  __syncthreads();
  {
    const double *bx = P.bxy + (int64_t)(4 * c + qd) * P.pl; const double czc = P.cz[c];
#pragma unroll
    for (int a = 0; a < NACC; ++a) {
      const int tr = a < NL ? w : XT, tc = a < NL ? a : w, par = tc >= HT ? 1 : 0;
      const double *lamz = P.lam_z[c][par];
      const double bxy = bx[min(b * HC + 16 * (tc - par * HT) + j, P.pl - 1)];
#pragma unroll
      for (int q = 0; q < 4; ++q) {
        const double den = fma(czc, lamz[16 * tr + 4 * q + kq], bxy);
        double r = __builtin_amdgcn_rcp(den);
        r = den < 1e300 ? fma(r, fma(-den, r, 1.0), r) : 0.0;
        L[(16 * tr + 4 * q + kq) * LD + 16 * tc + j] = acc[a][q] * r;
        __builtin_amdgcn_sched_barrier(0);
      }
    }
  }
  zero_acc();
  __syncthreads();
  gemm(std::integral_constant<int, NCH>{}, P.kk2);
  auto put = [&](int row, int col, double a, double bb) {
    if (row >= R || col >= C) return;
    const int mr = P.ng - 1 - row;
    const double vlo = mr == row ? a : a + bb, vhi = a - bb;
#pragma unroll
    for (int t = 0; t < 2; ++t) { const int64_t d0 = dst[2 * row + t]; if (d0 >= 0) out[d0 + cb + col] = vlo; }
    if (mr != row) {
#pragma unroll
      for (int t = 0; t < 2; ++t) { const int64_t d1 = dst[2 * mr + t]; if (d1 >= 0) out[d1 + cb + col] = vhi; }
    }
  };
#pragma unroll
  for (int u = 0; u < HT; ++u) {
#pragma unroll
    for (int q = 0; q < 4; ++q) put(16 * w + 4 * q + kq, 16 * u + j, acc[u][q], acc[u + HT][q]);
  }
  if constexpr (EXTRA) {
    __syncthreads();
    if (pw) {
#pragma unroll
      for (int q = 0; q < 4; ++q) L[((w - HT) * 4 + q) * 64 + lane] = acc[NL][q];
    }
    __syncthreads();
    if (!pw) {
#pragma unroll
      for (int q = 0; q < 4; ++q) put(16 * XT + 4 * q + kq, 16 * w + j, acc[NL][q], L[(w * 4 + q) * 64 + lane]);
    }
  }
}
template <int NT> void launch_zpass_both(hipStream_t s, const OctPass &P, const int64_t *dst, int n_items, const double *in, double *out, hipEvent_t e0, hipEvent_t e1) {
  hipExtLaunchKernelGGL((k_fdmo_zpass_both<NT>), dim3((unsigned)n_items), dim3(64 * (NT < 4 ? NT : 4)), 0, s, e0, e1, 0, P, dst, in, out);
}

template <auto Kernel, int NT, class Elem> void launch_one(hipStream_t s, int n_items, const OctPass &P, const double *in, double *out, hipEvent_t e0, hipEvent_t e1) {
  constexpr unsigned lds = (unsigned)(PassGeom<NT>::PADN * PassGeom<NT>::LDMAX * sizeof(Elem));
  if (lds > 64 * 1024) {
    static std::mutex mu; static std::set<int> done; int dev = 0; PORO_HIP(hipGetDevice(&dev));
    std::lock_guard<std::mutex> lk(mu);
    if (!done.count(dev)) { PORO_HIP(hipFuncSetAttribute(reinterpret_cast<const void *>(Kernel), hipFuncAttributeMaxDynamicSharedMemorySize, (int)lds)); done.insert(dev); }
  }
  hipExtLaunchKernelGGL(Kernel, dim3((unsigned)n_items), dim3(64 * pass_waves<NT>()), lds, s, e0, e1, 0, P, in, out);
}
enum class PassVariant { Octant, SlabU, General, OctantF32, PerDirection };
constexpr const char *kVariantName[] = {"Octant", "SlabU", "General", "OctantF32", "PerDirection"};
PassVariant variant_of_flags(const OctPass &P) {
  const bool plain = P.vec2 == 1 && !P.use_in_off && !P.use_out_off && P.bxy_cmul == 4;
  const bool unit = P.vec2 == 1 && !P.use_in_off && !P.use_out_off && P.slab_z == 0 && P.slab_io == 0 && !P.row_in;
  if (P.per_dir) return unit && P.bxy_cmul >= 1 && P.bxy_cmul <= 4 && P.no_shift >= 0 && P.no_shift < 3 ? PassVariant::PerDirection : PassVariant::General;
  const bool oct = plain && P.slab_z == 0 && P.slab_io == 0 && !P.row_in && P.no_shift == 3;
  const bool slab_u = plain && P.no_shift == 2 && ((P.mode == 0 && P.slab_io == 1 && !P.slab_z) || (P.mode == 1 && P.slab_z == 2 && P.row_in && !P.slab_io) || (P.mode == 2 && P.slab_io == 2 && !P.slab_z));
  return oct ? PassVariant::Octant : slab_u ? PassVariant::SlabU : PassVariant::General;
}
template <int NT, int VAR> void launch_modes(hipStream_t s, const OctPass &P, int n_items, const double *in, double *out, hipEvent_t e0, hipEvent_t e1) {
  if (P.mode == 0) launch_one<k_fdmo_pass<NT, 0, VAR>, NT, double>(s, n_items, P, in, out, e0, e1);
  else if (P.mode == 2) launch_one<k_fdmo_pass<NT, 2, VAR>, NT, double>(s, n_items, P, in, out, e0, e1);
  else if ((VAR == 0 || VAR == 3) && P.gz_part) launch_one<k_fdmo_pass<NT, 1, (VAR == 3 ? 3 : 0), true>, NT, double>(s, n_items, P, in, out, e0, e1);
  else launch_one<k_fdmo_pass<NT, 1, VAR>, NT, double>(s, n_items, P, in, out, e0, e1);
}
template <int NT> void launch_pass(hipStream_t s, PassVariant v, const OctPass &P, int n_items, const double *in, double *out, hipEvent_t e0, hipEvent_t e1) {
  switch (v) {
    case PassVariant::Octant: launch_modes<NT, 0>(s, P, n_items, in, out, e0, e1); break;
    case PassVariant::SlabU: launch_modes<NT, 1>(s, P, n_items, in, out, e0, e1); break;
    case PassVariant::General: launch_modes<NT, 2>(s, P, n_items, in, out, e0, e1); break;
    case PassVariant::PerDirection: launch_modes<NT, 3>(s, P, n_items, in, out, e0, e1); break;
    case PassVariant::OctantF32:
      if (P.mode == 0) launch_one<k_fdmo_pass_f32<NT, 0>, NT, float>(s, n_items, P, in, out, e0, e1);
      else if (P.mode == 2) launch_one<k_fdmo_pass_f32<NT, 2>, NT, float>(s, n_items, P, in, out, e0, e1);
      else if (P.gz_part) launch_one<k_fdmo_pass_f32<NT, 1, true>, NT, float>(s, n_items, P, in, out, e0, e1);
      else launch_one<k_fdmo_pass_f32<NT, 1>, NT, float>(s, n_items, P, in, out, e0, e1);
      break;
  }
}
void launch_pass_nt(hipStream_t s, int nt, PassVariant v, const OctPass &P, int n_blocks, const double *in, double *out, hipEvent_t e0 = nullptr, hipEvent_t e1 = nullptr) {
  const PassVariant flags = variant_of_flags(P);
  if (flags != (v == PassVariant::OctantF32 ? PassVariant::Octant : v)) throw Error(std::string("fdmo: pass stated as ") + kVariantName[(int)v] + ", the flags of its descriptor are those of " + kVariantName[(int)flags]);
  switch (nt) {
    case 1: launch_pass<1>(s, v, P, n_blocks, in, out, e0, e1); break;
    case 2: launch_pass<2>(s, v, P, n_blocks, in, out, e0, e1); break;
    case 3: launch_pass<3>(s, v, P, n_blocks, in, out, e0, e1); break;
    case 4: launch_pass<4>(s, v, P, n_blocks, in, out, e0, e1); break;
    case 5: launch_pass<5>(s, v, P, n_blocks, in, out, e0, e1); break;
    case 6: launch_pass<6>(s, v, P, n_blocks, in, out, e0, e1); break;
    case 7: launch_pass<7>(s, v, P, n_blocks, in, out, e0, e1); break;
    case 8: launch_pass<8>(s, v, P, n_blocks, in, out, e0, e1); break;
    default: throw Error("fdmo: half lines of more than 128 entries");
  }
}
inline int pass2_chunk(int nt) { return nt == 5 ? 64 : 16 * nt; }
inline int pass2_chunks(int pl, int nt) { return (pl + pass2_chunk(nt) - 1) / pass2_chunk(nt); }
inline int oct_grid(int64_t co, int nc = 3) { return (int)std::min<int64_t>((nc * co + kBlock - 1) / kBlock, kMaxPartials); }
inline int split_mask_of(const FdmOct &O) { return O.per_dir ? O.split_mask : O.no == 8 ? 7 : O.no == 4 ? 3 : 0; }
OctDims dims_of(const FdmOct &O) {
  OctDims D{O.n[0], O.n[1], O.n[2], O.h[0], O.h[1], O.h[2], O.hxp, O.co_stride, O.no, O.own_z, O.nc, split_mask_of(O), {}};
  for (int o = 0; o < 8; ++o) {
    int part = 0, k = 0;
    for (int d = 0; d < 3; ++d) if (D.split & (1 << d)) part |= ((o >> d) & 1) << k++;
    D.part[o] = (o & ~D.split) ? -1 : part;
  }
  return D;
}
SlabGeo geo_of(const FdmOct &O) { const auto &S = O.slab; return SlabGeo{S.cw, S.nchunk, S.cps, S.nb * S.nchunk, S.rank, S.my_chunks, S.hzg, S.ng, S.np, S.scols, (int64_t)O.hxp * O.h[1], O.co_stride}; }

struct Form {
  const FdmOct &O; bool scalar, f32;
  int pitch, blocks, no_shift;
  int nc, np, vec2, bxy_cmul;
  double kappa; const double *bxy;
  int hx() const { return O.h[0]; } int hy() const { return O.h[1]; } int planes() const { return O.h[2]; }
  int zlen() const { return O.slab.on ? O.slab.hzg : O.h[2]; } int cw() const { return O.slab.on ? O.slab.cw : pass2_chunk(O.nt_z); }
  int slot(int d, int p) const { return O.per_dir && !(O.split_mask & (1 << d)) ? 0 : p; }
  int bit(int d) const { int k = 0; for (int e = 0; e < d; ++e) k += (split_mask_of(O) >> e) & 1; return k; }
  const void *fwd(int c, int d, int p) const { c = scalar ? 0 : c; p = slot(d, p); return f32 ? (const void *)O.fwd32[c][d][p].p : (const void *)O.fwd[c][d][p].p; }
  const void *bwd(int c, int d, int p) const { c = scalar ? 0 : c; p = slot(d, p); return f32 ? (const void *)O.bwd32[c][d][p].p : (const void *)O.bwd[c][d][p].p; }
  const double *lam_z(int c, int p) const { return O.lam[scalar ? 0 : c][2][slot(2, p)].p; } double cz(int c) const { return scalar ? kappa : O.coef[c][2]; }
};
Form disp_form(const FdmOct &O, bool f32) {
  if (O.per_dir) { int ns = 0; for (int d = 0; d < 3; ++d) ns += (O.split_mask >> d) & 1; return Form{O, false, false, O.hxp, 3 * O.no, ns, 3, 2, 1, 1 << ((O.split_mask & 1) + ((O.split_mask >> 1) & 1)), 0.0, O.bxy.p}; }
  return Form{O, false, f32, O.hxp, 3 * O.no, O.slab.on ? 2 : 3, 3, 2, 1, 4, 0.0, O.bxy.p};
}
Form scalar_form(const FdmOct &O, int nb, double kappa, const double *table) { return Form{O, true, false, O.h[0], nb, 0, nb, 1, 0, 0, kappa, table}; }
OctPass plan_pass(const Form &F, int pass) {
  auto ksteps = [](int n) { return (n + 3) / 4; };
  const int hx = F.hx(), hy = F.hy(), zlen = F.zlen(), cw = F.cw(), pl = F.pitch * hy; const bool first = pass == 1, transposed = F.O.slab.on;
  OctPass P{};
  if (F.O.per_dir) {
    P.per_dir = 1; P.bitz = F.bit(2);
  }
  const int bx = F.O.per_dir ? F.bit(0) : 0, by = F.O.per_dir ? F.bit(1) : 1, bz = F.O.per_dir ? F.bit(2) : 2;
  P.co_stride = F.O.co_stride; P.pl = pl; P.bxy = F.bxy; P.vec2 = F.vec2; P.no_shift = F.no_shift; P.bxy_cmul = F.bxy_cmul;
  if (pass == 2) {
    P.mode = 1; P.R = zlen; P.C = cw; P.kk1 = P.kk2 = ksteps(zlen); P.bit1 = P.bit2 = bz;
    P.nblk = transposed ? 1 : pass2_chunks(pl, F.O.nt_z); P.blk_stride = transposed ? (int64_t)zlen * cw : cw; P.row_stride = transposed ? cw : pl;
  } else {
    P.mode = first ? 0 : 2; P.R = hy; P.C = F.pitch; P.kk1 = ksteps(first ? hx : hy); P.kk2 = ksteps(first ? hy : hx); P.bit1 = first ? bx : by; P.bit2 = first ? by : bx;
    P.nblk = F.planes(); P.blk_stride = pl; P.row_stride = F.pitch;
  }
  for (int c = 0; c < F.nc; ++c) {
    P.cz[c] = F.cz(c);
    for (int p = 0; p < F.np; ++p) {
      P.lam_z[c][p] = F.lam_z(c, p);
      if (pass == 1) { P.T1[c][p] = F.fwd(c, 0, p); P.T2[c][p] = F.fwd(c, 1, p); }
      else if (pass == 2) { P.T1[c][p] = F.fwd(c, 2, p); P.T2[c][p] = F.bwd(c, 2, p); }
      else { P.T1[c][p] = F.bwd(c, 1, p); P.T2[c][p] = F.bwd(c, 0, p); }
    }
  }
  return P;
}
OctPass plan_slab_pass(const Form &F, int pass) {
  const auto &S = F.O.slab;
  OctPass P = plan_pass(F, pass);
  if (pass == 2) {
    P.slab_z = S.np; P.chunk0 = S.chunk0; P.chunk_total = S.nb * S.nchunk; P.nchunk = S.nchunk; P.row_in = S.row_in.p; P.ng = S.ng;
    P.vec2 = 1;
  } else {
    const bool first = pass == 1;
    P.slab_io = first ? 1 : 2; P.store_planes = S.own; P.scols = (int)S.scols; P.inv_scols = 1.0f / (float)S.scols; P.col_unit = S.nchunk * S.cw; P.rank = S.rank;
    P.dest_stride = (int64_t)((first ? S.max_own : S.max_nl) - 1) * S.scols; P.recv_off = S.recv_off;
  }
  return P;
}
struct PassStamps {
  bool on = false; DevBuf<unsigned long long> buf; int items[3] = {0, 0, 0};
  static const char *path() { static const char *p = std::getenv("PORO_FDMO_STAMPS"); return p; }
  PassStamps() { static int calls = 0; on = path() && ++calls == 3; }
  void attach(hipStream_t s, OctPass (&P)[3], const int (&n_items)[3]) {
    if (!on) return;
    buf.alloc((size_t)8 * (n_items[0] + n_items[1] + n_items[2])); buf.zero(s);
    for (int k = 0, at = 0; k < 3; at += n_items[k++]) { items[k] = n_items[k]; P[k].stamps = buf.p + 8 * (int64_t)at; }
  }
  void dump(hipStream_t s) {
    if (!on) return;
    PORO_HIP(hipStreamSynchronize(s));
    std::vector<unsigned long long> h(buf.n); PORO_HIP(hipMemcpy(h.data(), buf.p, buf.n * sizeof(unsigned long long), hipMemcpyDeviceToHost));
    FILE *f = std::fopen(path(), "w"); const unsigned long long *r = h.data();
    for (int pass = 0; f && pass < 3; ++pass) for (int b = 0; b < items[pass]; ++b, r += 8) std::fprintf(f, "%d %d %llu %llu %llu %llu %llu %llu %llu %llu\n", pass, b, r[0], r[1], r[2], r[3], r[4], r[5], r[6], r[7]);
    if (f) std::fclose(f);
  }
};
void form_geometry(FdmOct &O, const int nn[3], const double (*coef)[3], int nsplit, int no, hipStream_t s) {
  const int zline = O.slab.on ? O.slab.ng : nn[2]; int hmax = nsplit ? (zline + 1) / 2 : zline;
  for (int d = 0; d < 3; ++d) {
    O.n[d] = nn[d]; O.h[d] = d < nsplit ? (nn[d] + 1) / 2 : nn[d];
    if (d < 2) hmax = std::max(hmax, O.h[d]);
    for (int c = 0; coef && c < 3; ++c) O.coef[c][d] = coef[c][d];
  }
  O.nt = O.nt_z = (hmax + 15) / 16; O.hxp = nsplit ? (O.h[0] + 1) & ~1 : O.h[0]; O.no = no;
  O.co_stride = (int64_t)O.hxp * O.h[1] * O.h[2]; O.n_oct = (coef ? 3 : 1) * no * O.co_stride;
  if (coef) { O.g.alloc(O.n_oct); O.z.alloc(O.n_oct); O.t.alloc(O.n_oct); O.g.zero(s); O.z.zero(s); O.t.zero(s); }
}
void slab_prologue(FdmOct &O, const int nn[3], int rank, const std::vector<int> &node_layers, const char *who) {
  auto &S = O.slab; const int N = (int)node_layers.size();
  S.on = true; S.n_ranks = N; S.rank = rank;
  S.ng = 1; for (int q = 0; q < N; ++q) S.ng += node_layers[q];
  if (nn[2] != node_layers[rank] + 1) throw Error(std::string(who) + ": local planes do not match the layer table");
}

}

struct FdmoPlans { OctPass pass[2][3]; int n_items[3]; };

bool fdmo_usable(int dim, const int nn[3]) {
  if (dim != 3) return false;
  for (int d = 0; d < 3; ++d) if ((nn[d] + 1) / 2 > 16 * kFdmoMaxTiles || nn[d] < 2) return false;
  return true;
}

void fdmo_init(FdmOct &O, const int nn[3], const double coef[3][3], hipStream_t s) {
  form_geometry(O, nn, coef, 3, 8, s);
  const int64_t n_u = (int64_t)3 * nn[0] * nn[1] * nn[2];
  if (n_u > O.n_oct) throw Error("fdmo_init: the octant array is smaller than the nodal vector");
  O.own_z = O.n[2];
  O.gz_n = 24 * pass2_chunks(O.hxp * O.h[1], O.nt);
  O.gz_part.alloc(O.gz_n); O.gz_part.zero(s);
}
void fdmo_init_per_direction(FdmOct &O, const int nn[3], const double coef[3][3], const FdmFormDecision &D, hipStream_t s) {
  if (!D.usable) throw Error("fdmo_init_per_direction: a line of more than 128 entries");
  O.per_dir = true; O.split_mask = 0; O.no = 1;
  for (int d = 0; d < 3; ++d) {
    O.n[d] = nn[d]; O.h[d] = D.len[d];
    if (D.split[d]) { O.split_mask |= 1 << d; O.no *= 2; }
    for (int c = 0; c < 3; ++c) O.coef[c][d] = coef[c][d];
  }
  O.nt = D.nt_xy; O.nt_z = D.nt_z; O.hxp = (O.h[0] + 1) & ~1;
  O.co_stride = (int64_t)O.hxp * O.h[1] * O.h[2]; O.n_oct = (int64_t)3 * O.no * O.co_stride;
  if ((int64_t)3 * nn[0] * nn[1] * nn[2] > O.n_oct) throw Error("fdmo_init_per_direction: the form's array is smaller than the nodal vector");
  if (O.hxp > 16 * O.nt || O.h[1] > 16 * O.nt || O.h[2] > 16 * O.nt_z) throw Error("fdmo_init_per_direction: tile counts do not cover the lines");
  O.g.alloc(O.n_oct); O.z.alloc(O.n_oct); O.t.alloc(O.n_oct); O.g.zero(s); O.z.zero(s); O.t.zero(s);
  O.own_z = O.n[2];
  O.gz_n = 3 * O.no * pass2_chunks(O.hxp * O.h[1], O.nt_z);
  O.gz_part.alloc(O.gz_n); O.gz_part.zero(s);
}
static void slab_layout(FdmOct &O, int nb, int np, int rank, const std::vector<int> &node_layers, hipStream_t s) {
  auto &S = O.slab; const int N = (int)node_layers.size();
  S.nb = nb; S.np = np; S.hzg = np == 2 ? (S.ng + 1) / 2 : S.ng;
  const int64_t pl = (int64_t)O.hxp * O.h[1];
  S.zboth = np == 2 && (O.nt == 2 || O.nt == 4 || O.nt == 5) && !std::getenv("PORO_FDMO_SLAB_TWO_PARITY_WORKGROUPS");
  S.cw = S.zboth ? pass2_chunk(O.nt) / 2 : pass2_chunk(O.nt); S.nchunk = (int)((pl + S.cw - 1) / S.cw);
  const int chunk_total = nb * S.nchunk;
  S.cps = (chunk_total + N - 1) / N; S.chunk0 = rank * S.cps; S.my_chunks = std::max(0, std::min(S.cps, chunk_total - S.chunk0)); S.scols = (int64_t)S.cps * S.cw;
  std::vector<int> off(N), own(N), nl(N); int acc = 0; S.max_own = S.max_nl = S.rows_back = 0;
  for (int q = 0; q < N; ++q) { off[q] = acc; acc += node_layers[q]; own[q] = node_layers[q] + (q == N - 1 ? 1 : 0); nl[q] = node_layers[q] + 1; S.max_own = std::max(S.max_own, own[q]); S.max_nl = std::max(S.max_nl, nl[q]); S.rows_back += nl[q]; }
  S.own = own[rank]; S.nl = nl[rank];
  if ((int64_t)std::max(S.max_own, S.max_nl) * chunk_total * S.cw >= (int64_t)1 << 31 || (int64_t)S.rows_back * S.scols >= (int64_t)1 << 31 || (int64_t)chunk_total * S.cw >= (int64_t)1 << 24) throw Error("fdmo: a slab of more than 2^31 transform entries");
  const int64_t blk = (int64_t)std::max(S.max_own, S.max_nl) * S.scols; S.recv_off = blk * N;
  std::vector<int64_t> rin(S.ng), rout(S.rows_back); std::vector<int32_t> rkz(S.rows_back);
  for (int q = 0; q < N; ++q) for (int k = 0; k < own[q]; ++k) rin[off[q] + k] = S.recv_off + ((int64_t)q * S.max_own + k) * S.scols;
  { int r = 0; for (int q = 0; q < N; ++q) for (int k = 0; k < nl[q]; ++k, ++r) { rout[r] = ((int64_t)q * S.max_nl + k) * S.scols + (q == rank ? S.recv_off : 0); rkz[r] = off[q] + k; } }
  S.row_in.upload(rin); S.row_out.upload(rout); S.row_kz.upload(rkz);
  { std::vector<int64_t> d2((size_t)2 * S.ng, -1);
    for (int r = 0; r < S.rows_back; ++r) { const int kz = rkz[r]; d2[2 * kz + (d2[2 * kz] >= 0 ? 1 : 0)] = rout[r]; }
    S.dst2.upload(d2); }
  S.buf.alloc((size_t)2 * blk * N); S.buf.zero(s);
  if (!S.zboth) { S.tz.alloc((size_t)np * S.cps * S.hzg * S.cw); S.tz.zero(s); }
}
void fdmo_init_slab(FdmOct &O, const int nn[3], const double coef[3][3], int rank, const std::vector<int> &node_layers, bool has_upper, hipStream_t s) {
  slab_prologue(O, nn, rank, node_layers, "fdmo_init_slab");
  form_geometry(O, nn, coef, 2, 4, s);
  O.own_z = has_upper ? nn[2] - 1 : nn[2];
  slab_layout(O, 12, 2, rank, node_layers, s);
}
void fdmo_scalar_init_slab(FdmOct &O, const int nn[3], int rank, const std::vector<int> &node_layers, hipStream_t s) {
  slab_prologue(O, nn, rank, node_layers, "fdmo_scalar_init_slab");
  form_geometry(O, nn, nullptr, 0, 1, s);
  slab_layout(O, 1, 1, rank, node_layers, s);
}

static void fdmo_upload_dir_whole(FdmOct &O, int comp, int dir, const LineTables &T) {
  const int nt = dir == 2 ? O.nt_z : O.nt;
  std::vector<double> lp(16 * nt + 16, std::numeric_limits<double>::infinity());
  for (int m = 0; m < T.n; ++m) lp[m] = T.lam[m];
  O.h_lam[comp][dir][0] = lp; O.lam[comp][dir][0].upload(lp);
  O.fwd[comp][dir][0].upload(whole_line_fragments(T, nt, false)); O.bwd[comp][dir][0].upload(whole_line_fragments(T, nt, true));
}
void fdmo_upload_dir(FdmOct &O, int comp, int dir, const LineTables &T) {
  if (O.per_dir && T.n != O.n[dir]) throw Error("fdmo_upload_dir: line length mismatch");
  if (O.per_dir && !(O.split_mask & (1 << dir))) { fdmo_upload_dir_whole(O, comp, dir, T); return; }
  const int nn = T.n, h = (nn + 1) / 2, nt = dir == 2 ? O.nt_z : O.nt, padn = 16 * nt;
  const std::vector<double> &S = T.S, &lam = T.lam;
  if (nn != (O.slab.on && dir == 2 ? O.slab.ng : O.n[dir])) throw Error("fdmo_upload_dir: line length mismatch");
  if (!T.parity) throw Error("fdmo_upload_dir: tables whose modes are not all even or odd");
  const std::vector<int> *const grp[2] = {&T.even, &T.odd};
  for (int p = 0; p < 2; ++p) {
    const std::vector<int> &g = *grp[p]; const int ng = (int)g.size();
    const std::vector<double> F = pack_fragments<double>(nt, 4 * nt, ng, h, [&](int r, int cc) { return S[(size_t)cc * nn + g[r]]; }), B = pack_fragments<double>(nt, 4 * nt, h, ng, [&](int r, int cc) { return S[(size_t)r * nn + g[cc]]; });
    std::vector<double> lp(padn + 16, std::numeric_limits<double>::infinity());
    for (int m = 0; m < ng; ++m) lp[m] = lam[g[m]];
    O.h_lam[comp][dir][p] = lp;
    O.fwd[comp][dir][p].upload(F); O.bwd[comp][dir][p].upload(B); O.lam[comp][dir][p].upload(lp);
    if (!O.slab.on && !O.per_dir) {
      O.fwd32[comp][dir][p].upload(std::vector<float>(F.begin(), F.end())); O.bwd32[comp][dir][p].upload(std::vector<float>(B.begin(), B.end()));
    }
  }
}

void fdmo_finalize(FdmOct &O) {
  const int hx = O.h[0], hy = O.h[1], hxp = O.hxp; const size_t pl = (size_t)hxp * hy;
  const int sx = O.per_dir ? (O.split_mask & 1) : 1, sy = O.per_dir ? ((O.split_mask >> 1) & 1) : 1, cmul = 1 << (sx + sy);
  std::vector<double> B((size_t)3 * cmul * pl, 1.0);
  for (int c = 0; c < 3; ++c) for (int q = 0; q < cmul; ++q) for (int my = 0; my < hy; ++my) for (int mx = 0; mx < hx; ++mx) {
    const int px = sx ? q & 1 : 0, py = sy ? (q >> sx) & 1 : 0;
    B[(size_t)(cmul * c + q) * pl + (size_t)my * hxp + mx] = O.coef[c][0] * O.h_lam[c][0][px][mx] + O.coef[c][1] * O.h_lam[c][1][py][my];
  }
  O.bxy.upload(B);
  auto plans = std::make_shared<FdmoPlans>();
  for (int f32 = 0; f32 < (O.slab.on || O.per_dir ? 1 : 2); ++f32) for (int k = 0; k < 3; ++k) {
    const Form F = disp_form(O, f32 != 0);
    plans->pass[f32][k] = O.slab.on ? plan_slab_pass(F, k + 1) : plan_pass(F, k + 1);
    plans->n_items[k] = F.blocks * plans->pass[f32][k].nblk;
  }
  O.plans = plans;
}

void fdmo_apply(hipStream_t s, const FdmOct &O, const double *g_oct, double *z_oct, double *scratch, const PcgScalars *gate, hipEvent_t *ev, double *gz_part, int precision, const PcgStopTest &stop) {
  const bool f32 = precision == PORO_FDM_FP32;
  if (f32 && (O.slab.on || O.planar || O.per_dir || !O.fwd32[0][0][0].p)) throw Error("fdmo_apply: fp32 transforms exist for the single-rank octant form only");
  OctPass P[3]; const int (&n_items)[3] = O.plans->n_items;
  for (int k = 0; k < 3; ++k) { P[k] = O.plans->pass[f32][k]; P[k].gate = gate; }
  if (gz_part && n_items[1] != O.gz_n) throw Error("fdmo_apply: the g.z partial buffer does not match the grid of pass 2");
  P[1].gz_part = gz_part;
  P[0].stop = stop;
  if (stop.gg_part && stop.sc != gate) throw Error("fdmo_apply: a stopping test without the gate of its solve");
  PassStamps stamps; stamps.attach(s, P, n_items);
  if (f32 && !scratch) throw Error("fdmo_apply: the fp32 transforms need the scratch array");
  double *const mid = scratch ? scratch : z_oct;
  const double *const in[3] = {g_oct, mid, mid}; double *const out[3] = {mid, mid, z_oct};
  for (int k = 0; k < 3; ++k) launch_pass_nt(s, k == 1 ? O.nt_z : O.nt, f32 ? PassVariant::OctantF32 : O.per_dir ? PassVariant::PerDirection : PassVariant::Octant, P[k], n_items[k], in[k], out[k], ev ? ev[2 * k] : nullptr, ev ? ev[2 * k + 1] : nullptr);
  stamps.dump(s);
}

void fdmo_slab_pass(hipStream_t s, const FdmOct &O, int pass, const double *in, double *out, const PcgScalars *gate, hipEvent_t e0, hipEvent_t e1) {
  const auto &S = O.slab;
  OctPass P = O.plans->pass[0][pass - 1]; P.gate = gate;
  if (pass != 2) launch_pass_nt(s, O.nt, PassVariant::SlabU, P, O.plans->n_items[pass - 1], in, out, e0, e1);
  else if (S.my_chunks <= 0) return;
  else if (!S.zboth) launch_pass_nt(s, O.nt, PassVariant::SlabU, P, 2 * S.my_chunks, in, out, e0, e1);
  else switch (O.nt) {
    case 2: launch_zpass_both<2>(s, P, S.dst2.p, S.my_chunks, in, out, e0, e1); break;
    case 4: launch_zpass_both<4>(s, P, S.dst2.p, S.my_chunks, in, out, e0, e1); break;
    case 5: launch_zpass_both<5>(s, P, S.dst2.p, S.my_chunks, in, out, e0, e1); break;
    default: throw Error("fdmo: both-parity z pass needs 2, 4 or 5 tiles per half line");
  }
}
static int copy_grid(int64_t n) { return (int)std::max<int64_t>(1, std::min<int64_t>((n + 255) / 256, 4096)); }
void fdmo_slab_scatter_pack(hipStream_t s, const FdmOct &O, const PcgScalars *gate) {
  const auto &S = O.slab; const SlabGeo G = geo_of(O);
  if (S.my_chunks > 0) hipLaunchKernelGGL(k_fdmo_slab_scatter_pack, copy_grid((int64_t)S.rows_back * S.my_chunks * S.cw), 256, 0, s, G, S.rows_back, S.row_out.p, S.row_kz.p, S.tz.p, S.buf.p, gate);
}
void fdmo_dot_owned(hipStream_t s, const FdmOct &O, const double *a, const double *b, double *partials, const PcgScalars *gate) {
  hipLaunchKernelGGL(k_fdmo_dot_owned, std::max(oct_grid(O.co_stride, O.nc), O.nc * O.no), kBlock, 0, s, dims_of(O), a, b, partials, gate);
}

bool fdmo_scalar_usable(int dim, const int nn[3]) { if (dim != 3) return false; for (int d = 0; d < 3; ++d) if (nn[d] > 16 * kFdmoMaxTiles || nn[d] < 2) return false; return true; }
void fdmo_scalar_init(FdmOct &O, const int nn[3], hipStream_t s) {
  form_geometry(O, nn, nullptr, 0, 1, s);
  O.t.alloc(3 * O.n_oct); O.t.zero(s);
}
void fdmo_scalar_upload_dir(FdmOct &O, int dir, const LineTables &T) {
  const int n = T.n; const std::vector<double> &S = T.S, &lam = T.lam;
  if (n != (O.slab.on && dir == 2 ? O.slab.ng : O.n[dir])) throw Error("fdmo_scalar_upload_dir: line length mismatch");
  std::vector<double> lp(16 * O.nt + 16, std::numeric_limits<double>::infinity());
  for (int m = 0; m < n; ++m) lp[m] = lam[m];
  O.h_lam[0][dir][0] = lp; O.lam[0][dir][0].upload(lp);
  O.fwd[0][dir][0].upload(pack_fragments<double>(O.nt, 4 * O.nt, n, n, [&](int r, int cc) { return S[(size_t)cc * n + r]; })); O.bwd[0][dir][0].upload(pack_fragments<double>(O.nt, 4 * O.nt, n, n, [&](int r, int cc) { return S[(size_t)r * n + cc]; }));
}
static const double *scalar_table(hipStream_t s, FdmOct &O, double a, double kappa);
int fdmo_scalar_apply(hipStream_t s, FdmOct &O, double a, double kappa, const double *g, double *z, const PcgScalars *gate) {
  const double *gs[1] = {g}; double *zs[1] = {z};
  return fdmo_scalar_apply_many(s, O, a, kappa, 1, gs, zs, gate);
}
template <int NT, int MODE> void launch_strip_one(hipStream_t s, int n_wg, const OctPass &P, const double *in, double *out) {
  constexpr unsigned lds = (unsigned)(PassGeom<NT>::PADN * (MODE == 1 ? 16 : PassGeom<NT>::LDMAX) * sizeof(double));
  if (lds > 64 * 1024) {
    static std::mutex mu; static std::set<int> done; int dev = 0; PORO_HIP(hipGetDevice(&dev));
    std::lock_guard<std::mutex> lk(mu);
    if (!done.count(dev)) { PORO_HIP(hipFuncSetAttribute(reinterpret_cast<const void *>(k_fdmo_strip<NT, MODE>), hipFuncAttributeMaxDynamicSharedMemorySize, (int)lds)); done.insert(dev); }
  }
  hipLaunchKernelGGL((k_fdmo_strip<NT, MODE>), dim3((unsigned)n_wg), dim3(64 * NT), lds, s, P, in, out);
}
template <int NT> void launch_strip(hipStream_t s, const OctPass &P, int n_items, const double *in, double *out) {
  if (P.mode == 0) launch_strip_one<NT, 0>(s, n_items * NT, P, in, out);
  else if (P.mode == 2) launch_strip_one<NT, 2>(s, n_items * NT, P, in, out);
  else launch_strip_one<NT, 1>(s, n_items, P, in, out);
}
void launch_strip_nt(hipStream_t s, int nt, const OctPass &P, int n_items, const double *in, double *out) {
  if (variant_of_flags(P) != PassVariant::General || P.slab_z || P.slab_io || P.row_in || P.no_shift || P.bxy_cmul || P.stop.gg_part || P.gz_part || P.stamps) throw Error("fdmo: the strip form serves the scalar passes of one rank only");
  switch (nt) {
    case 2: launch_strip<2>(s, P, n_items, in, out); break;
    case 3: launch_strip<3>(s, P, n_items, in, out); break;
    case 4: launch_strip<4>(s, P, n_items, in, out); break;
    case 5: launch_strip<5>(s, P, n_items, in, out); break;
    case 6: launch_strip<6>(s, P, n_items, in, out); break;
    case 7: launch_strip<7>(s, P, n_items, in, out); break;
    case 8: launch_strip<8>(s, P, n_items, in, out); break;
    default: throw Error("fdmo: lines of more than 128 entries");
  }
}
int fdmo_scalar_apply_many(hipStream_t s, FdmOct &O, double a, double kappa, int nb, const double *const *g, double *const *z, const PcgScalars *gate) {
  if (nb < 1 || nb > 3) throw Error("fdmo_scalar_apply_many: 1..3 right-hand sides");
  const Form F = scalar_form(O, nb, kappa, scalar_table(s, O, a, kappa));
  const double *const in[3] = {g[0], O.t.p, O.t.p}; double *const out[3] = {O.t.p, O.t.p, z[0]};
  int strips = 0;
  for (int k = 0; k < 3; ++k) {
    OctPass P = plan_pass(F, k + 1);
    P.gate = gate;
    for (int c = 0; c < nb; ++c) { P.in_blk[c] = g[c]; P.out_blk[c] = z[c]; }
    P.use_in_off = k == 0; P.use_out_off = k == 2;
    const bool strip = O.nt >= 2 && !O.slab.on && (double)nb * P.nblk < O.strip_limit && g[0] != O.t.p && z[0] != O.t.p;
    if (!strip) { launch_pass_nt(s, O.nt, PassVariant::General, P, nb * P.nblk, in[k], out[k]); continue; }
    if (k == 1) { P.C = 16; P.blk_stride = 16; P.nblk = (P.pl + 15) / 16; }
    launch_strip_nt(s, O.nt, P, nb * P.nblk, in[k], out[k]);
    ++strips;
  }
  return strips;
}

static const double *scalar_table(hipStream_t s, FdmOct &O, double a, double kappa) {
  for (auto &T : O.scalar_tables) if (T.a == a && T.kappa == kappa) return T.t.p;
  const int hx = O.h[0], hy = O.h[1];
  if (O.scalar_tables.size() >= 8) { PORO_HIP(hipStreamSynchronize(s)); O.scalar_tables.pop_front(); }
  std::vector<double> Bt((size_t)hx * hy);
  const double inf = std::numeric_limits<double>::infinity();
  for (int my = 0; my < hy; ++my) for (int mx = 0; mx < hx; ++mx) {
    const double lx = O.h_lam[0][0][0][mx], ly = O.h_lam[0][1][0][my];
    Bt[(size_t)my * hx + mx] = (lx < 1e300 && ly < 1e300) ? a + kappa * (lx + ly) : inf;
  }
  O.scalar_tables.emplace_back(); auto &T = O.scalar_tables.back(); T.a = a; T.kappa = kappa; T.t.upload(Bt); return T.t.p;
}
void fdmo_scalar_slab_pass(hipStream_t s, FdmOct &O, int pass, double a, double kappa, const double *in, double *out) {
  const Form F = scalar_form(O, 1, kappa, scalar_table(s, O, a, kappa));
  const OctPass P = plan_slab_pass(F, pass);
  const int n_items = pass == 2 ? O.slab.my_chunks : P.nblk;
  if (n_items > 0) launch_pass_nt(s, O.nt, PassVariant::General, P, n_items, in, out);
}

#define PORO_OCT_LAUNCH(kernel, O, ...) do { if ((O).nc == 2) hipLaunchKernelGGL((kernel<2, false>), oct_grid((O).co_stride, 2), kBlock, 0, s, dims_of(O), __VA_ARGS__); \
                                              else if ((O).per_dir) hipLaunchKernelGGL((kernel<3, true>), oct_grid((O).co_stride, 3), kBlock, 0, s, dims_of(O), __VA_ARGS__); \
                                              else hipLaunchKernelGGL((kernel<3, false>), oct_grid((O).co_stride, 3), kBlock, 0, s, dims_of(O), __VA_ARGS__); } while (0)
bool fdmo_planar_usable(int dim, const int nn[3]) { return dim == 2 && nn[0] >= 2 && nn[1] >= 2 && nn[0] <= 4096 && nn[1] <= 4096; }
void fdmo_init_planar(FdmOct &O, const int nn[3], const double coef[3][3], hipStream_t s, bool split) {
  O.nc = 2; O.no = split ? 4 : 1; O.planar = true;
  for (int d = 0; d < 3; ++d) { O.n[d] = d < 2 ? nn[d] : 1; O.h[d] = d < 2 ? (split ? (nn[d] + 1) / 2 : nn[d]) : 1; for (int c = 0; c < 3; ++c) O.coef[c][d] = coef[c][d]; }
  O.nt = 0; O.hxp = (O.h[0] + 1) & ~1; O.own_z = 1;
  O.co_stride = (int64_t)O.hxp * O.h[1]; O.n_oct = 2 * O.no * O.co_stride;
  O.g.alloc(O.n_oct); O.z.alloc(O.n_oct); O.t.alloc(2 * O.n_oct);
  O.g.zero(s); O.z.zero(s); O.t.zero(s);
}
void fdmo_upload_dir_planar(FdmOct &O, int comp, int dir, const LineTables &T) {
  const int nn = T.n; const std::vector<double> &S = T.S, &lam = T.lam;
  if (nn != O.n[dir]) throw Error("fdmo_upload_dir_planar: line length mismatch");
  if (O.no == 1) {
    std::vector<double> F((size_t)nn * nn, 0.0), lp((size_t)nn + 16, std::numeric_limits<double>::infinity());
    for (int m = 0; m < nn; ++m) { if (!(lam[m] < 1e300)) continue; for (int k = 0; k < nn; ++k) F[(size_t)m * nn + k] = S[(size_t)k * nn + m]; lp[m] = lam[m]; }
    O.h_lam[comp][dir][0] = lp; O.fwd[comp][dir][0].upload(F); O.lam[comp][dir][0].upload(lp);
    return;
  }
  const int h = (nn + 1) / 2;
  if (!T.parity) throw Error("fdmo_upload_dir_planar: tables whose modes are not all even or odd");
  const std::vector<int> *const grp[2] = {&T.even, &T.odd};
  for (int p = 0; p < 2; ++p) {
    std::vector<double> F((size_t)h * h, 0.0), lp((size_t)h + 16, std::numeric_limits<double>::infinity());
    const std::vector<int> &g = *grp[p]; const int ng = (int)g.size();
    for (int m = 0; m < ng; ++m) { for (int k = 0; k < h; ++k) F[(size_t)m * h + k] = S[(size_t)k * nn + g[m]]; lp[m] = lam[g[m]]; }
    O.h_lam[comp][dir][p] = lp; O.fwd[comp][dir][p].upload(F); O.lam[comp][dir][p].upload(lp);
  }
}
void fdmo_apply_planar(hipStream_t s, const FdmOct &O, const double *g, double *z, const PcgScalars *gate, const PcgStopTest &stop) {
  const int hx = O.h[0], hy = O.h[1], hxp = O.hxp; const int64_t co = O.co_stride;
  double *t1 = O.t.p, *t2 = O.t.p + O.n_oct;
  const int no = O.no, nb = 2 * no;
  if (stop.gg_part && stop.sc != gate) throw Error("fdmo_apply_planar: a stopping test without the gate of its solve");
  Gemm2D G{}; G.nb = nb; G.gate = gate; G.rsC = hxp; G.stop = stop;
  auto launch = [&](bool ak, bool bk) {
    const dim3 grid((unsigned)(((G.M + 63) / 64) * ((G.N + 63) / 64)), (unsigned)nb);
    if (ak && bk) hipLaunchKernelGGL((k_fdmo_gemm2d<true, true>), grid, 256, 0, s, G);
    else if (ak) hipLaunchKernelGGL((k_fdmo_gemm2d<true, false>), grid, 256, 0, s, G);
    else hipLaunchKernelGGL((k_fdmo_gemm2d<false, false>), grid, 256, 0, s, G);
  };
  G.M = hy; G.N = hx; G.K = hx; G.rsA = hxp; G.csA = 1; G.rsB = 1; G.csB = hx; G.scale = 0;
// ... 39 lines not shown
```

Measured before the change: 24.52 billion.

## Add class-split vertex/midpoint FDM transform passes for Q2 octant preconditioner

Adds an alternative fast-diagonalisation path for Q2 displacement lines. Each 1D eigenbasis is split into vertex and midpoint node classes with a 2x2 mixing per frequency, so each pass multiplies by smaller class matrices instead of the full line transform. New host code builds and verifies the class tables, and new kernels plus plans and launchers implement the three passes. The path is on by default when the tables validate and can be turned off with an env var. It adds complexity and a second code path whose kernels differ from the tuned ones, for example the z pass uses O.nt rather than nt_z.

```diff
diff --git a/poroelasticity_dealii_amd/csrc/common.hpp b/poroelasticity_dealii_amd/csrc/common.hpp
--- a/poroelasticity_dealii_amd/csrc/common.hpp
+++ b/poroelasticity_dealii_amd/csrc/common.hpp
@@ -111,6 +111,8 @@
     DevBuf<int64_t> row_out; DevBuf<int32_t> row_kz;
     DevBuf<double> buf, tz;
   } slab;
+  bool class_split = false;
+  DevBuf<double> cfwd[3][3][2][2], cbwd[3][3][2][2], cmix[3][3][2], clam[3][3][2], bxy_vm; std::vector<double> h_clam[3][3][2];
   std::shared_ptr<FdmoPlans> plans;
   struct ScalarTable { double a, kappa; DevBuf<double> t; };
   std::list<ScalarTable> scalar_tables;
@@ -390,6 +392,8 @@
 void fdmo_init_slab(FdmOct &O, const int nn[3], const double coef[3][3], int rank, const std::vector<int> &node_layers, bool has_upper, hipStream_t s);
 void fdmo_init_per_direction(FdmOct &O, const int nn[3], const double coef[3][3], const FdmFormDecision &D, hipStream_t s);
 void fdmo_upload_dir(FdmOct &O, int comp, int dir, const LineTables &T);
+void fdmo_upload_dir_classes(FdmOct &O, int comp, int dir, const ClassSplitTables &T);
+bool fdmo_class_split_runs(const FdmOct &O, int precision);
 void fdmo_finalize(FdmOct &O);
 void fdmo_apply(hipStream_t s, const FdmOct &O, const double *g_oct, double *z_oct, double *scratch_oct, const PcgScalars *gate = nullptr, hipEvent_t *ev  = nullptr,
                 double *gz_part  = nullptr,
diff --git a/poroelasticity_dealii_amd/csrc/ctx_prec.hip b/poroelasticity_dealii_amd/csrc/ctx_prec.hip
--- a/poroelasticity_dealii_amd/csrc/ctx_prec.hip
+++ b/poroelasticity_dealii_amd/csrc/ctx_prec.hip
@@ -283,7 +283,7 @@
     F.sendbuf.alloc(blk * N); F.recvbuf.alloc(blk * N); F.tz1.alloc((size_t)dim * F.ng * F.C); F.tz2.alloc((size_t)dim * F.ng * F.C);
     F.sendbuf.zero(c->stream); F.recvbuf.zero(c->stream); F.tz1.zero(c->stream); F.tz2.zero(c->stream);
   }
-  LineTables tables[3][4]; bool same_ends[3], parity[3], parity_cd[3][3] = {};
+  LineTables tables[3][4]; ClassSplitTables classes[3][4]; bool same_ends[3], parity[3], parity_cd[3][3] = {};
   const auto key_of = [&](int comp, int d) { return F.fix[comp][d][0] * 2 + F.fix[comp][d][1]; };
   for (int d = 0; d < dim; ++d) {
     if (line && d == last) { same_ends[d] = parity[d] = false; continue; }
@@ -311,7 +311,17 @@
     }
     if (per_dir) { fdmo_init_per_direction(c->fdm_oct, nn3, F.coef, form, c->stream); oct_ok = true; }
     else if (oct_ok && planar) fdmo_init_planar(c->fdm_oct, nn3, F.coef, c->stream, symmetric);
-    else if (oct_ok && !multi) fdmo_init(c->fdm_oct, nn3, F.coef, c->stream);
+    else if (oct_ok && !multi) {
+      fdmo_init(c->fdm_oct, nn3, F.coef, c->stream);
+      const char *hook = std::getenv("PORO_FDMO_CLASS_SPLIT");
+      bool all = !(hook && std::atoi(hook) == 0);
+      for (int d = 0; d < dim && all; ++d) for (int comp = 0; comp < dim && all; ++comp) {
+        ClassSplitTables &CS = classes[d][key_of(comp, d)];
+        if (!CS.n) CS = class_split_tables(ku, c->lines.hcell[d], F.fix[comp][d][0] != 0, F.fix[comp][d][1] != 0, tables[d][key_of(comp, d)]);
+        all = all && CS.ok;
+      }
+      c->fdm_oct.class_split = all;
+    }
     if (oct_ok && multi) { std::vector<int> node_layers(F.n_ranks); for (int q = 0; q < F.n_ranks; ++q) node_layers[q] = ku * F.layers[q];
                            fdmo_init_slab(c->fdm_oct, nn3, F.coef, F.rank, node_layers, c->comm.part.has_upper != 0, c->stream); } }
   for (int d = 0; d < dim; ++d) for (int comp = 0; comp < dim; ++comp) {
@@ -321,6 +331,7 @@
     FdmuDir &D = global_dir ? F.last_global[comp] : F.dir[comp][d];
     if (!(planar && oct_ok && T.n > 320 && !same_ends[d])) fdmu_upload_dir(D, T, global_dir ? false : F.single, same_ends[d] && parity[d]);
     if (oct_ok) { if (planar) fdmo_upload_dir_planar(c->fdm_oct, comp, d, T); else fdmo_upload_dir(c->fdm_oct, comp, d, T); }
+    if (oct_ok && c->fdm_oct.class_split) fdmo_upload_dir_classes(c->fdm_oct, comp, d, classes[d][key_of(comp, d)]);
   }
   c->fdmu_t1.alloc(c->n_u); c->fdmu_t2.alloc(c->n_u); c->fdmu_t1.zero(c->stream); c->fdmu_t2.zero(c->stream);
   if (!c->wz_u.p) { c->wz_u.alloc(c->n_u); c->wz_u.zero(c->stream); }
@@ -368,6 +379,7 @@
   if (O.slab.on) { if (stop.gg_part) throw Error("fdm_precondition_u_form: the slab form runs no stopping test"); fdm_precondition_u_slab(c, g, z, gate); return false; }
   if (O.planar) { fdmo_apply_planar(c->stream, O, g, z, gate, stop); return false; }
   const char *names[3] = {"fdm_u_pass1", "fdm_u_pass2", "fdm_u_pass3"};
+  if (fdmo_class_split_runs(O, precision)) c->timers["fdm_u_class_split"].enqueued++;
   if (!begin_sampled_dispatch(c, names[0])) {
     fdmo_apply(c->stream, O, g, z, scratch, gate, nullptr, gz_part, precision, stop);
     return gz_part != nullptr;
diff --git a/poroelasticity_dealii_amd/csrc/fdm_tables.hpp b/poroelasticity_dealii_amd/csrc/fdm_tables.hpp
--- a/poroelasticity_dealii_amd/csrc/fdm_tables.hpp
+++ b/poroelasticity_dealii_amd/csrc/fdm_tables.hpp
@@ -244,6 +244,113 @@
                   : pack_fragments<double>(tiles, 4 * tiles, n, n, [&](int r, int c) { return S[(size_t)c * n + r]; });
 }
 
+struct ClassSplitGroup {
+  int nv = 0, nm = 0;
+  int slots = 0;
+  std::vector<double> Fv, Fm;
+  std::vector<double> mix;
+  std::vector<double> lam_v, lam_m;
+};
+struct ClassSplitTables {
+  bool ok = false; const char *why = ""; int n = 0; ClassSplitGroup grp[2];
+  double off_block = 0, orth = 0, resid = 0, eig_dev = 0;
+};
+inline ClassSplitTables class_split_tables(int k, const std::vector<double> &hc, bool fix_lo, bool fix_hi, const LineTables &T) {
+  ClassSplitTables R; const int N = (int)hc.size(), nn = 2 * N + 1, h = (nn + 1) / 2; R.n = nn;
+  if (k != 2) { R.why = "no midpoint class (not Q2)"; return R; }
+  if (T.n != nn || !T.parity || fix_lo != fix_hi) { R.why = "modes without parity"; return R; }
+  const bool fix = fix_lo; const double pi = 3.14159265358979323846, kTol = 1e-12;
+  std::vector<double> M, K; fe1d(2, hc, M, K);
+  auto band = [&](const std::vector<double> &A, const std::vector<double> &x, std::vector<double> &y) {
+    y.assign(nn, 0.0);
+    for (int i = 0; i < nn; ++i) for (int p = std::max(0, i - 2); p <= std::min(nn - 1, i + 2); ++p) y[i] += A[(size_t)i * nn + p] * x[p];
+  };
+  auto dot = [&](const std::vector<double> &x, const std::vector<double> &y) { double s = 0; for (int i = 0; i < nn; ++i) s += x[i] * y[i]; return s; };
+  struct Vec { int m, cls; std::vector<double> v, Mv, Kv; };
+  std::vector<Vec> vecs; std::vector<int> at_v(N + 1, -1), at_m(N + 1, -1);
+  for (int m = fix ? 1 : 0; m <= N; ++m) for (int cls = 0; cls < 2; ++cls) {
+    Vec V; V.m = m; V.cls = cls; V.v.assign(nn, 0.0); double big = 0;
+    for (int i = cls; i < nn; i += 2) { V.v[i] = (fix && (i == 0 || i == nn - 1)) ? 0.0 : fix ? std::sin(m * pi * i / (2.0 * N)) : std::cos(m * pi * i / (2.0 * N)); big = std::max(big, std::fabs(V.v[i])); }
+    if (big < 1e-9) continue;
+    band(M, V.v, V.Mv); band(K, V.v, V.Kv);
+    (cls ? at_m : at_v)[m] = (int)vecs.size(); vecs.push_back(std::move(V));
+  }
+  const int nvec = (int)vecs.size();
+  { double big = 0, off = 0;
+    for (int w = 0; w < 2; ++w) {
+      double bw = 0, ow = 0;
+      for (int a = 0; a < nvec; ++a) for (int b = 0; b < nvec; ++b) {
+        const double e = std::fabs(dot(vecs[a].v, w ? vecs[b].Mv : vecs[b].Kv));
+        bw = std::max(bw, e); if (vecs[a].m != vecs[b].m) ow = std::max(ow, e);
+      }
+      big = std::max(big, bw); if (bw > 0) off = std::max(off, ow / bw);
+    }
+    R.off_block = off;
+    if (!(big > 0) || !(off <= kTol)) { R.why = "vertex / midpoint classes couple across frequencies"; return R; } }
+  for (int p = 0; p < 2; ++p) { R.grp[p].nv = (h + 1) / 2; R.grp[p].nm = h / 2; }
+  std::vector<std::vector<double>> Fcol; std::vector<double> Flam; const double inf = std::numeric_limits<double>::infinity();
+  for (int m = fix ? 1 : 0; m <= N; ++m) {
+    const int ia = at_v[m], ib = at_m[m];
+    if (ia < 0 && ib < 0) continue;
+    const std::vector<double> &ref = vecs[ia >= 0 ? ia : ib].v;
+    double ds = 0, da = 0;
+    for (int i = 0; i < nn; ++i) { const double a = ref[i], b = ref[nn - 1 - i]; ds += (a - b) * (a - b); da += (a + b) * (a + b); }
+    if (std::min(ds, da) > 1e-20 * std::max(ds, da)) { R.why = "a class vector is neither even nor odd"; return R; }
+    ClassSplitGroup &G = R.grp[ds <= da ? 0 : 1]; const int s = G.slots++;
+    G.Fv.resize((size_t)G.slots * G.nv, 0.0); G.Fm.resize((size_t)G.slots * G.nm, 0.0); G.mix.resize((size_t)G.slots * 4, 0.0); G.lam_v.resize(G.slots, inf); G.lam_m.resize(G.slots, inf);
+    if (ia >= 0) for (int q = 0; q < G.nv; ++q) G.Fv[(size_t)s * G.nv + q] = vecs[ia].v[2 * q];
+    if (ib >= 0) for (int q = 0; q < G.nm; ++q) G.Fm[(size_t)s * G.nm + q] = vecs[ib].v[2 * q + 1];
+    double *w = &G.mix[(size_t)s * 4];
+    if (ia >= 0 && ib >= 0) {
+      const double maa = dot(vecs[ia].v, vecs[ia].Mv), mab = dot(vecs[ia].v, vecs[ib].Mv), mbb = dot(vecs[ib].v, vecs[ib].Mv);
+      const double kr[2][2] = {{dot(vecs[ia].v, vecs[ia].Kv), dot(vecs[ia].v, vecs[ib].Kv)}, {dot(vecs[ib].v, vecs[ia].Kv), dot(vecs[ib].v, vecs[ib].Kv)}};
+      if (!(maa > 0)) { R.why = "class mass block not positive definite"; return R; }
+      const double l11 = std::sqrt(maa), l21 = mab / l11, d2 = mbb - l21 * l21;
+      if (!(d2 > 0)) { R.why = "class mass block not positive definite"; return R; }
+      const double l22 = std::sqrt(d2);
+      double X[2][2], Z[2][2];
+      for (int j = 0; j < 2; ++j) { X[0][j] = kr[0][j] / l11; X[1][j] = (kr[1][j] - l21 * X[0][j]) / l22; }
+      for (int j = 0; j < 2; ++j) { Z[0][j] = X[j][0] / l11; Z[1][j] = (X[j][1] - l21 * Z[0][j]) / l22; }
+      std::vector<double> C = {Z[0][0], 0.5 * (Z[0][1] + Z[1][0]), 0.5 * (Z[0][1] + Z[1][0]), Z[1][1]}, Q, lam;
+      jacobi_eig(2, C, Q, lam);
+      const int jv = lam[0] <= lam[1] ? 0 : 1, jm = 1 - jv;
+      const int js[2] = {jv, jm};
+      for (int e = 0; e < 2; ++e) { const double q0 = Q[js[e]], q1 = Q[2 + js[e]], w1 = q1 / l22, w0 = (q0 - l21 * w1) / l11; w[2 * e] = w0; w[2 * e + 1] = w1; }
+      G.lam_v[s] = std::max(lam[jv], 0.0); G.lam_m[s] = std::max(lam[jm], 0.0);
+    } else if (ia >= 0) { const double maa = dot(vecs[ia].v, vecs[ia].Mv); w[0] = 1.0 / std::sqrt(maa); G.lam_v[s] = std::max(dot(vecs[ia].v, vecs[ia].Kv) / maa, 0.0); }
+    else { const double mbb = dot(vecs[ib].v, vecs[ib].Mv); w[3] = 1.0 / std::sqrt(mbb); G.lam_m[s] = std::max(dot(vecs[ib].v, vecs[ib].Kv) / mbb, 0.0); }
+    for (int e = 0; e < 2; ++e) {
+      const double lam_e = e ? G.lam_m[s] : G.lam_v[s];
+      if (!(lam_e < 1e300)) continue;
+      std::vector<double> f(nn, 0.0);
+      for (int i = 0; i < nn; ++i) f[i] = (ia >= 0 ? w[2 * e] * vecs[ia].v[i] : 0.0) + (ib >= 0 ? w[2 * e + 1] * vecs[ib].v[i] : 0.0);
+      Fcol.push_back(std::move(f)); Flam.push_back(lam_e);
+    }
+  }
+  const int nmode = (int)Fcol.size(); double lam_max = 0; for (double v : Flam) lam_max = std::max(lam_max, v);
+  int nfree = 0; std::vector<double> ref; for (int j = 0; j < nn; ++j) if (T.lam[j] < 1e300) { ++nfree; ref.push_back(T.lam[j]); lam_max = std::max(lam_max, T.lam[j]); }
+  if (nmode != nfree || !(lam_max > 0)) { R.why = "mode count differs from the line's"; return R; }
+  { std::vector<double> Mf, Kf;
+    for (int b = 0; b < nmode; ++b) {
+      band(M, Fcol[b], Mf); band(K, Fcol[b], Kf);
+      for (int a = 0; a < nmode; ++a) {
+        R.orth = std::max(R.orth, std::fabs(dot(Fcol[a], Mf) - (a == b ? 1.0 : 0.0)));
+        R.resid = std::max(R.resid, std::fabs(dot(Fcol[a], Kf) - (a == b ? Flam[a] : 0.0)) / lam_max);
+      }
+    }
+    if (!(R.orth <= kTol) || !(R.resid <= kTol)) { R.why = "class-split eigenvectors do not diagonalise the pencil"; return R; } }
+  { std::vector<double> mine = Flam; std::sort(mine.begin(), mine.end()); std::sort(ref.begin(), ref.end());
+    for (int j = 0; j < nmode; ++j) R.eig_dev = std::max(R.eig_dev, std::fabs(mine[j] - ref[j]) / lam_max);
+    if (!(R.eig_dev <= kTol)) { R.why = "eigenvalues differ from the line's"; return R; } }
+  for (int p = 0; p < 2; ++p) if (R.grp[p].slots > std::max(R.grp[p].nv, R.grp[p].nm)) { R.why = "more frequencies than class positions"; return R; }
+  R.ok = true; return R;
+}
+inline std::vector<double> class_fragments(const ClassSplitGroup &G, int cls, int tiles, int ksteps, bool backward) {
+  const std::vector<double> &F = cls ? G.Fm : G.Fv; const int np = cls ? G.nm : G.nv, ns = G.slots;
+  return backward ? pack_fragments<double>(tiles, ksteps, np, ns, [&](int r, int c) { return F[(size_t)c * np + r]; })
+                  : pack_fragments<double>(tiles, ksteps, ns, np, [&](int r, int c) { return F[(size_t)r * np + c]; });
+}
+
 constexpr int kFdmoMaxTiles = 8;
 struct FdmFormDecision { bool usable = false, all_split = false; int split[3] = {0, 0, 0}, len[3] = {0, 0, 0}; int nt_xy = 0, nt_z = 0, parts = 1; };
 inline FdmFormDecision fdm_form_decide(const int fix[3][3][2], const bool parity[3][3] , const int nn[3]) {
diff --git a/poroelasticity_dealii_amd/csrc/kernels_fdmo.hip b/poroelasticity_dealii_amd/csrc/kernels_fdmo.hip
--- a/poroelasticity_dealii_amd/csrc/kernels_fdmo.hip
+++ b/poroelasticity_dealii_amd/csrc/kernels_fdmo.hip
@@ -460,6 +460,255 @@
   }
 }
 
+struct OctPassVM {
+  int mode, R, C, nblk, pl;
+  int64_t co_stride, blk_stride, row_stride;
+  int bit1, bit2;
+  int kkv[2], kkm[2];
+  int nvx, nvy, nmy;
+  const double *Tv[2][3][2], *Tm[2][3][2];
+  const double *mix[2][3][2];
+  const double *lam_z[3][2];
+  double cz[3]; const double *bxy;
+  double *gz_part; const PcgScalars *gate; PcgStopTest stop;
+};
+template <int NT> constexpr int vm_waves() { return NT == 5 ? 4 : (NT + 1) / 2; }
+template <int NT> constexpr int vm_waves_per_simd() { return NT <= 5 ? 3 : NT == 6 ? 2 : 1; }
+template <int NT, int MODE, bool GZ = false>
+__global__ void __launch_bounds__(64 * vm_waves<NT>()) __attribute__((amdgpu_waves_per_eu(vm_waves_per_simd<NT>())))
+k_fdmo_pass_vm(OctPassVM P, const double *in, double *out) {
+  static_assert(!GZ || MODE == 1, "g . z comes out of pass 2");
+  typedef PassGeom<NT> Gm;
+  constexpr bool QUAD = NT == 5;
+  constexpr int NW = vm_waves<NT>(), NCT = (NT + 1) / 2, H = 8 * NT, KK = 2 * NT, PADN = Gm::PADN;
+  constexpr int NB = MODE == 1 ? (NT == 5 ? 4 : NT) : NT;
+  constexpr bool kColsFirst = MODE == 0, kColsSecond = MODE == 2;
+  constexpr int LD1 = kColsFirst ? Gm::LDA : Gm::LDB, LD2 = kColsSecond ? Gm::LDA : Gm::LDB;
+  extern __shared__ double L[];
+  __shared__ double gz_wave[GZ ? NW : 1];
+  if (MODE == 0 && P.stop.gg_part) {
+    PcgStopInputs stop_in;
+    pcg_stop_load(P.stop, stop_in);
+    if (P.gate && (P.gate->done | P.gate->finishing)) return;
+    if (pcg_stop_decide(P.stop, stop_in)) return;
+  } else if (pcg_gate_closed(P.gate)) return;
+  const int tid = threadIdx.x, lane = tid & 63, w = __builtin_amdgcn_readfirstlane(tid >> 6);
+  const int j = lane & 15, kq = lane >> 4;
+  const int co = blockIdx.x / P.nblk, b = blockIdx.x % P.nblk, c = co >> 3, o = co & 7;
+  const int64_t base = (int64_t)co * P.co_stride + (int64_t)b * P.blk_stride;
+  const int R = P.R, C = MODE == 1 ? min(P.C, P.pl - b * P.C) : P.C;
+  const int p1 = (o >> P.bit1) & 1, p2 = (o >> P.bit2) & 1;
+  auto node_of = [](int r) { return r < H ? 2 * r : 2 * (r - H) + 1; };
+  if constexpr (MODE == 0) {
+    constexpr int TOT = PADN * H, PER = (TOT + 64 * NW - 1) / (64 * NW);
+    double2 stage[PER];
+#pragma unroll
+    for (int u = 0; u < PER; ++u) {
+      const int e = tid + u * 64 * NW, r = e / H, cp = e - r * H, rn = node_of(r);
+      stage[u] = (e < TOT && rn < R && 2 * cp < C) ? *reinterpret_cast<const double2 *>(in + base + (int64_t)rn * P.row_stride + 2 * cp) : double2{0.0, 0.0};
+    }
+#pragma unroll
+    for (int u = 0; u < PER; ++u) { const int e = tid + u * 64 * NW, r = e / H, cp = e - r * H; if (e < TOT) { L[r * LD1 + cp] = stage[u].x; L[r * LD1 + H + cp] = stage[u].y; } }
+  } else if constexpr (MODE == 1) {
+    constexpr int HP = 8 * NB, TOT = PADN * HP, PER = (TOT + 64 * NW - 1) / (64 * NW);
+    double2 stage[PER];
+#pragma unroll
+    for (int u = 0; u < PER; ++u) {
+      const int e = tid + u * 64 * NW, r = e / HP, c2 = 2 * (e - r * HP), rn = node_of(r);
+      stage[u] = (e < TOT && rn < R && c2 < C) ? *reinterpret_cast<const double2 *>(in + base + (int64_t)rn * P.row_stride + c2) : double2{0.0, 0.0};
+    }
+#pragma unroll
+    for (int u = 0; u < PER; ++u) { const int e = tid + u * 64 * NW, r = e / HP, c2 = 2 * (e - r * HP); if (e < TOT) *reinterpret_cast<double2 *>(&L[r * LD1 + c2]) = stage[u]; }
+  } else {
+    constexpr int TOT = H * H, PER = (TOT + 64 * NW - 1) / (64 * NW);
+    const int nvx = P.nvx, nmx = C - P.nvx, nvy = P.nvy, nmy = P.nmy;
+    const double *__restrict__ my = P.mix[0][c][p1], *__restrict__ mx = P.mix[1][c][p2];
+    double stage[PER][4];
+#pragma unroll
+    for (int u = 0; u < PER; ++u) {
+      const int e = tid + u * 64 * NW, sy = e / H, sx = e - sy * H;
+      const bool ok = e < TOT, rv = ok && sy < nvy, rm = ok && sy < nmy, cv = sx < nvx, cm = sx < nmx;
+      const double *src = in + base + sx;
+      stage[u][0] = (rv && cv) ? src[(int64_t)sy * P.row_stride] : 0.0;
+      stage[u][1] = (rv && cm) ? src[(int64_t)sy * P.row_stride + nvx] : 0.0;
+      stage[u][2] = (rm && cv) ? src[(int64_t)(nvy + sy) * P.row_stride] : 0.0;
+      stage[u][3] = (rm && cm) ? src[(int64_t)(nvy + sy) * P.row_stride + nvx] : 0.0;
+    }
+#pragma unroll
+    for (int u = 0; u < PER; ++u) {
+      const int e = tid + u * 64 * NW, sy = e / H, sx = e - sy * H;
+      if (e < TOT) {
+        const double2 y0 = *reinterpret_cast<const double2 *>(my + 4 * sy), y1 = *reinterpret_cast<const double2 *>(my + 4 * sy + 2);
+        const double2 x0 = *reinterpret_cast<const double2 *>(mx + 4 * sx), x1 = *reinterpret_cast<const double2 *>(mx + 4 * sx + 2);
+        const double av_v = fma(y0.x, stage[u][0], y1.x * stage[u][2]), am_v = fma(y0.y, stage[u][0], y1.y * stage[u][2]);
+        const double av_m = fma(y0.x, stage[u][1], y1.x * stage[u][3]), am_m = fma(y0.y, stage[u][1], y1.y * stage[u][3]);
+        L[sy * LD1 + sx] = fma(x0.x, av_v, x1.x * av_m); L[sy * LD1 + H + sx] = fma(x0.y, av_v, x1.y * av_m);
+        L[(H + sy) * LD1 + sx] = fma(x0.x, am_v, x1.x * am_m); L[(H + sy) * LD1 + H + sx] = fma(x0.y, am_v, x1.y * am_m);
+      }
+    }
+  }
+  constexpr int NA = QUAD ? 4 : NB, NACC = (QUAD && MODE == 1) ? NCT : NA, NTF = QUAD ? NCT : 1;
+  const bool roleB = QUAD && (MODE == 1 || w == NW - 1);
+  const int fixed = roleB ? (MODE == 1 ? w : NB - 1) : w;
+  auto tile_of = [&](int a, int &ct, int &bt) { ct = roleB ? a : fixed; bt = roleB ? fixed : a; return a < (roleB ? NCT : NA); };
+  constexpr int CHK = 2, NCH = KK / CHK;
+  const double *__restrict__ T1v = P.Tv[0][c][p1] + lane, *__restrict__ T1m = P.Tm[0][c][p1] + lane, *__restrict__ T2v = P.Tv[1][c][p2] + lane, *__restrict__ T2m = P.Tm[1][c][p2] + lane;
+  double tf[2][2][CHK][NTF];
+  auto load_chunk = [&](auto role_c, int buf, int step) {
+    constexpr bool RB = decltype(role_c)::value;
+    const double *__restrict__ Tv = step < NCH ? T1v : T2v, *__restrict__ Tm = step < NCH ? T1m : T2m; const int ch = step < NCH ? step : step - NCH;
+#pragma unroll
+    for (int k = 0; k < CHK; ++k) {
+#pragma unroll
+      for (int f = 0; f < (RB ? NCT : 1); ++f) { const int ct = RB ? f : fixed; tf[buf][0][k][f] = Tv[((int64_t)ct * KK + CHK * ch + k) * 64]; tf[buf][1][k][f] = Tm[((int64_t)ct * KK + CHK * ch + k) * 64]; }
+    }
+  };
+  v4d accv[NACC], accm[NACC];
+  auto zero_acc = [&]() {
+#pragma unroll
+    for (int t = 0; t < NACC; ++t) { accv[t] = v4d{0, 0, 0, 0}; accm[t] = v4d{0, 0, 0, 0}; }
+  };
+  auto gemm = [&](auto role_c, auto contract_cols, auto ld_c, auto first_step_c, int kkv, int kkm) {
+    constexpr bool RB = decltype(role_c)::value, kCols = decltype(contract_cols)::value; constexpr int LD = decltype(ld_c)::value, S0 = decltype(first_step_c)::value;
+    constexpr int ND = RB ? 1 : NA, NF = RB ? NCT : 1;
+    const double *La = (kCols ? L + j * LD + kq : L + kq * LD + j) + (RB ? (kCols ? 16 * fixed * LD : 16 * fixed) : 0);
+#pragma unroll
+    for (int kk = 0; kk < KK; ++kk) {
+      const int buf = (S0 + kk / CHK) & 1;
+#pragma unroll
+      for (int cls = 0; cls < 2; ++cls) {
+        if (kk < (cls ? kkm : kkv)) {
+          double d[ND];
+#pragma unroll
+          for (int t = 0; t < ND; ++t) d[t] = kCols ? La[16 * t * LD + cls * H + 4 * kk] : La[(cls * H + 4 * kk) * LD + 16 * t];
+#pragma unroll
+          for (int a = 0; a < (RB ? NF : ND); ++a) {
+            const double dv = d[RB ? 0 : a], tv = tf[buf][cls][kk % CHK][RB ? a : 0];
+            v4d &acc = cls ? accm[a] : accv[a];
+            acc = kCols ? __builtin_amdgcn_mfma_f64_16x16x4f64(dv, tv, acc, 0, 0, 0) : __builtin_amdgcn_mfma_f64_16x16x4f64(tv, dv, acc, 0, 0, 0);
+          }
+        }
+      }
+      if (kk % CHK == CHK - 1 && S0 + kk / CHK + 2 < ((MODE == 1 && S0 == 0) ? NCH : 2 * NCH)) load_chunk(role_c, buf, S0 + kk / CHK + 2);
+    }
+  };
+  auto by_role = [&](auto f) {
+    if constexpr (!QUAD) f(std::false_type{});
+    else if constexpr (MODE == 1) f(std::true_type{});
+    else { if (roleB) f(std::true_type{}); else f(std::false_type{}); }
+  };
+  typedef std::integral_constant<bool, kColsFirst> CF; typedef std::integral_constant<int, LD1> L1c;
+  typedef std::integral_constant<bool, kColsSecond> CS; typedef std::integral_constant<int, LD2> L2c;
+  typedef std::integral_constant<int, 0> S0c; typedef std::integral_constant<int, NCH> S1c;
+  by_role([&](auto r) { load_chunk(r, 0, 0); load_chunk(r, 1, 1); });
+  zero_acc();
+  __syncthreads();
+  by_role([&](auto r) { gemm(r, CF{}, L1c{}, S0c{}, P.kkv[0], P.kkm[0]); });
+  __syncthreads();
+  if constexpr (MODE == 0) {
+#pragma unroll
+    for (int a = 0; a < NACC; ++a) {
+      int ct, bt; if (!tile_of(a, ct, bt)) continue;
+      const int s = 16 * ct + j;
+      const double *__restrict__ m1 = P.mix[0][c][p1] + 4 * s;
+      const double2 w0 = *reinterpret_cast<const double2 *>(m1), w1 = *reinterpret_cast<const double2 *>(m1 + 2);
+      if (s < H) {
+#pragma unroll
+        for (int q = 0; q < 4; ++q) {
+          const double av = accv[a][q], bb = accm[a][q]; const int row = 16 * bt + 4 * q + kq;
+          L[row * LD2 + s] = fma(w0.x, av, w0.y * bb); L[row * LD2 + H + s] = fma(w1.x, av, w1.y * bb);
+        }
+      }
+    }
+  } else if constexpr (MODE == 2) {
+#pragma unroll
+    for (int a = 0; a < NACC; ++a) {
+      int ct, bt; if (!tile_of(a, ct, bt)) continue;
+#pragma unroll
+      for (int q = 0; q < 4; ++q) {
+        const int p = 16 * ct + 4 * q + kq;
+        if (p < H) { L[p * LD2 + 16 * bt + j] = accv[a][q]; L[(H + p) * LD2 + 16 * bt + j] = accm[a][q]; }
+      }
+    }
+  } else {
+    const double *__restrict__ lamz = P.lam_z[c][p1], *__restrict__ m1 = P.mix[0][c][p1];
+    const double *bx = P.bxy + (int64_t)(4 * c + (o & 3)) * P.pl; const double czc = P.cz[c];
+    double gz = 0;
+#pragma unroll
+    for (int a = 0; a < NACC; ++a) {
+      int ct, bt; if (!tile_of(a, ct, bt)) continue;
+      const double bxy = bx[min(b * P.C + 16 * bt + j, P.pl - 1)];
+#pragma unroll
+      for (int q = 0; q < 4; ++q) {
+        const int s = 16 * ct + 4 * q + kq;
+        const double2 w0 = *reinterpret_cast<const double2 *>(m1 + 4 * s), w1 = *reinterpret_cast<const double2 *>(m1 + 4 * s + 2);
+        const double lzv = lamz[s], lzm = lamz[64 + s];
+        const double av = accv[a][q], bb = accm[a][q];
+        const double gv = fma(w0.x, av, w0.y * bb), gm = fma(w1.x, av, w1.y * bb);
+        const double dv = fma(czc, lzv, bxy), dm = fma(czc, lzm, bxy);
+        double rv = __builtin_amdgcn_rcp(dv), rm = __builtin_amdgcn_rcp(dm);
+        rv = dv < 1e300 ? fma(rv, fma(-dv, rv, 1.0), rv) : 0.0; rm = dm < 1e300 ? fma(rm, fma(-dm, rm, 1.0), rm) : 0.0;
+        const double zv = gv * rv, zm = gm * rm;
+        if constexpr (GZ) gz = fma(gm, zm, fma(gv, zv, gz));
+        if (s < H) { L[s * LD2 + 16 * bt + j] = fma(w0.x, zv, w1.x * zm); L[(H + s) * LD2 + 16 * bt + j] = fma(w0.y, zv, w1.y * zm); }
+        __builtin_amdgcn_sched_barrier(0);
+      }
+    }
+    if constexpr (GZ) {
+      gz = wave_sum(gz);
+      if (lane == 0) gz_wave[w] = gz;
+    }
+  }
+  if constexpr (MODE == 1) by_role([&](auto r) { load_chunk(r, NCH & 1, NCH); load_chunk(r, (NCH + 1) & 1, NCH + 1); });
+  zero_acc();
+  __syncthreads();
+  if constexpr (GZ) {
+    if (tid == 0) { double t = 0; for (int k = 0; k < NW; ++k) t += gz_wave[k]; P.gz_part[blockIdx.x] = t; }
+  }
+  by_role([&](auto r) { gemm(r, CS{}, L2c{}, S1c{}, P.kkv[1], P.kkm[1]); });
+  if constexpr (MODE == 0) {
+    const double *__restrict__ m2 = P.mix[1][c][p2];
+    const int nvx = P.nvx, nvy = P.nvy, nmy = P.nmy;
+#pragma unroll
+    for (int a = 0; a < NACC; ++a) {
+      int ct, bt; if (!tile_of(a, ct, bt)) continue;
+      const int cpos = 16 * bt + j, col = cpos < H ? (cpos < nvx ? cpos : -1) : (cpos - H < C - nvx ? nvx + cpos - H : -1);
+#pragma unroll
+      for (int q = 0; q < 4; ++q) {
+        const int s = 16 * ct + 4 * q + kq;
+        const double2 w0 = *reinterpret_cast<const double2 *>(m2 + 4 * s), w1 = *reinterpret_cast<const double2 *>(m2 + 4 * s + 2);
+        const double av = accv[a][q], bb = accm[a][q];
+        if (col >= 0 && s < nvy) out[base + (int64_t)s * P.row_stride + col] = fma(w0.x, av, w0.y * bb);
+        if (col >= 0 && s < nmy) out[base + (int64_t)(nvy + s) * P.row_stride + col] = fma(w1.x, av, w1.y * bb);
+      }
+    }
+  } else if constexpr (MODE == 2) {
+#pragma unroll
+    for (int a = 0; a < NACC; ++a) {
+      int ct, bt; if (!tile_of(a, ct, bt)) continue;
+      const int px = 16 * ct + j;
+#pragma unroll
+      for (int q = 0; q < 4; ++q) {
+        const int rn = node_of(16 * bt + 4 * q + kq);
+        if (px < H && rn < R && 2 * px < C) *reinterpret_cast<double2 *>(out + base + (int64_t)rn * P.row_stride + 2 * px) = double2{accv[a][q], accm[a][q]};
+      }
+    }
+  } else {
+#pragma unroll
+    for (int a = 0; a < NACC; ++a) {
+      int ct, bt; if (!tile_of(a, ct, bt)) continue;
+#pragma unroll
+      for (int q = 0; q < 4; ++q) {
+        const int p = 16 * ct + 4 * q + kq, cc = 16 * bt + j;
+        if (p < H && cc < C) {
+          if (2 * p < R) out[base + (int64_t)(2 * p) * P.row_stride + cc] = accv[a][q];
+          if (2 * p + 1 < R) out[base + (int64_t)(2 * p + 1) * P.row_stride + cc] = accm[a][q];
+        }
+      }
+    }
+  }
+}
+
 template <int NT, int MODE>
 __global__ void __launch_bounds__(64 * NT)
 k_fdmo_strip(OctPass P, const double *in, double *out) {
@@ -982,6 +1231,31 @@
     default: throw Error("fdmo: half lines of more than 128 entries");
   }
 }
+template <int NT> void launch_vm(hipStream_t s, const OctPassVM &P, int n_items, const double *in, double *out, hipEvent_t e0, hipEvent_t e1) {
+  constexpr unsigned lds = (unsigned)(PassGeom<NT>::PADN * PassGeom<NT>::LDMAX * sizeof(double));
+  auto go = [&](auto kernel) {
+    if (lds > 64 * 1024) {
+      static std::mutex mu; static std::set<std::pair<int, const void *>> done; int dev = 0; PORO_HIP(hipGetDevice(&dev));
+      std::lock_guard<std::mutex> lk(mu);
+      if (!done.count({dev, reinterpret_cast<const void *>(kernel)})) { PORO_HIP(hipFuncSetAttribute(reinterpret_cast<const void *>(kernel), hipFuncAttributeMaxDynamicSharedMemorySize, (int)lds)); done.insert({dev, reinterpret_cast<const void *>(kernel)}); }
+    }
+    hipExtLaunchKernelGGL(kernel, dim3((unsigned)n_items), dim3(64 * vm_waves<NT>()), lds, s, e0, e1, 0, P, in, out);
+  };
+  if (P.mode == 0) go(k_fdmo_pass_vm<NT, 0>); else if (P.mode == 2) go(k_fdmo_pass_vm<NT, 2>); else if (P.gz_part) go(k_fdmo_pass_vm<NT, 1, true>); else go(k_fdmo_pass_vm<NT, 1>);
+}
+void launch_vm_nt(hipStream_t s, int nt, const OctPassVM &P, int n_items, const double *in, double *out, hipEvent_t e0 = nullptr, hipEvent_t e1 = nullptr) {
+  switch (nt) {
+    case 1: launch_vm<1>(s, P, n_items, in, out, e0, e1); break;
+    case 2: launch_vm<2>(s, P, n_items, in, out, e0, e1); break;
+    case 3: launch_vm<3>(s, P, n_items, in, out, e0, e1); break;
+    case 4: launch_vm<4>(s, P, n_items, in, out, e0, e1); break;
+    case 5: launch_vm<5>(s, P, n_items, in, out, e0, e1); break;
+    case 6: launch_vm<6>(s, P, n_items, in, out, e0, e1); break;
+    case 7: launch_vm<7>(s, P, n_items, in, out, e0, e1); break;
+    case 8: launch_vm<8>(s, P, n_items, in, out, e0, e1); break;
+    default: throw Error("fdmo: half lines of more than 128 entries");
+  }
+}
 inline int pass2_chunk(int nt) { return nt == 5 ? 64 : 16 * nt; }
 inline int pass2_chunks(int pl, int nt) { return (pl + pass2_chunk(nt) - 1) / pass2_chunk(nt); }
 inline int oct_grid(int64_t co, int nc = 3) { return (int)std::min<int64_t>((nc * co + kBlock - 1) / kBlock, kMaxPartials); }
@@ -1042,6 +1316,21 @@
   }
   return P;
 }
+OctPassVM plan_vm(const FdmOct &O, const OctPass &D, int pass) {
+  OctPassVM P{};
+  P.mode = D.mode; P.R = D.R; P.C = D.C; P.nblk = D.nblk; P.pl = D.pl; P.co_stride = D.co_stride; P.blk_stride = D.blk_stride; P.row_stride = D.row_stride; P.bit1 = D.bit1; P.bit2 = D.bit2;
+  const int dir[2] = {pass == 1 ? 0 : pass == 2 ? 2 : 1, pass == 1 ? 1 : pass == 2 ? 2 : 0}; const bool back[2] = {pass == 3, pass != 1};
+  for (int g = 0; g < 2; ++g) {
+    const int h = O.h[dir[g]]; P.kkv[g] = ((h + 1) / 2 + 3) / 4; P.kkm[g] = (h / 2 + 3) / 4;
+    for (int c = 0; c < 3; ++c) for (int p = 0; p < 2; ++p) {
+      P.Tv[g][c][p] = (back[g] ? O.cbwd : O.cfwd)[c][dir[g]][p][0].p; P.Tm[g][c][p] = (back[g] ? O.cbwd : O.cfwd)[c][dir[g]][p][1].p; P.mix[g][c][p] = O.cmix[c][dir[g]][p].p;
+    }
+  }
+  P.nvx = (O.h[0] + 1) / 2; P.nvy = (O.h[1] + 1) / 2; P.nmy = O.h[1] / 2;
+  for (int c = 0; c < 3; ++c) { P.cz[c] = O.coef[c][2]; for (int p = 0; p < 2; ++p) P.lam_z[c][p] = O.clam[c][2][p].p; }
+  P.bxy = O.bxy_vm.p;
+  return P;
+}
 OctPass plan_slab_pass(const Form &F, int pass) {
   const auto &S = F.O.slab;
   OctPass P = plan_pass(F, pass);
@@ -1093,7 +1382,7 @@
 
 }
 
-struct FdmoPlans { OctPass pass[2][3]; int n_items[3]; };
+struct FdmoPlans { OctPass pass[2][3]; int n_items[3]; OctPassVM vm[3]; };
 
 bool fdmo_usable(int dim, const int nn[3]) {
   if (dim != 3) return false;
@@ -1189,8 +1478,32 @@
   }
 }
 
+void fdmo_upload_dir_classes(FdmOct &O, int comp, int dir, const ClassSplitTables &T) {
+  if (!O.class_split || O.per_dir || O.slab.on || O.planar) throw Error("fdmo_upload_dir_classes: the class-split passes exist for the single-rank octant form only");
+  if (!T.ok || T.n != O.n[dir]) throw Error("fdmo_upload_dir_classes: a line that is not class-split");
+  const int nt = O.nt, tiles = (nt + 1) / 2, ksteps = 2 * nt, h = O.h[dir]; const double inf = std::numeric_limits<double>::infinity();
+  for (int p = 0; p < 2; ++p) {
+    const ClassSplitGroup &G = T.grp[p];
+    if (G.nv != (h + 1) / 2 || G.nm != h / 2 || G.nv > 8 * nt || G.slots > 8 * nt || G.slots > 64) throw Error("fdmo_upload_dir_classes: class sizes do not fit the pass kernel");
+    for (int cls = 0; cls < 2; ++cls) { O.cfwd[comp][dir][p][cls].upload(class_fragments(G, cls, tiles, ksteps, false)); O.cbwd[comp][dir][p][cls].upload(class_fragments(G, cls, tiles, ksteps, true)); }
+    std::vector<double> mix(4 * 64, 0.0), lam(2 * 64, inf);
+    for (int s = 0; s < G.slots; ++s) { for (int e = 0; e < 4; ++e) mix[4 * s + e] = G.mix[4 * s + e]; lam[s] = G.lam_v[s]; lam[64 + s] = G.lam_m[s]; }
+    O.cmix[comp][dir][p].upload(mix); O.clam[comp][dir][p].upload(lam); O.h_clam[comp][dir][p] = lam;
+  }
+}
+bool fdmo_class_split_runs(const FdmOct &O, int precision) { return O.class_split && precision != PORO_FDM_FP32 && !O.per_dir && !O.slab.on && !O.planar; }
+
 void fdmo_finalize(FdmOct &O) {
   const int hx = O.h[0], hy = O.h[1], hxp = O.hxp; const size_t pl = (size_t)hxp * hy;
+  if (O.class_split) {
+    const int nvx = (hx + 1) / 2, nvy = (hy + 1) / 2;
+    std::vector<double> B((size_t)12 * pl, 1.0);
+    for (int c = 0; c < 3; ++c) for (int q = 0; q < 4; ++q) for (int my = 0; my < hy; ++my) for (int mx = 0; mx < hx; ++mx) {
+      const std::vector<double> &lx = O.h_clam[c][0][q & 1], &ly = O.h_clam[c][1][q >> 1];
+      B[(size_t)(4 * c + q) * pl + (size_t)my * hxp + mx] = O.coef[c][0] * (mx < nvx ? lx[mx] : lx[64 + mx - nvx]) + O.coef[c][1] * (my < nvy ? ly[my] : ly[64 + my - nvy]);
+    }
+    O.bxy_vm.upload(B);
+  }
   const int sx = O.per_dir ? (O.split_mask & 1) : 1, sy = O.per_dir ? ((O.split_mask >> 1) & 1) : 1, cmul = 1 << (sx + sy);
   std::vector<double> B((size_t)3 * cmul * pl, 1.0);
   for (int c = 0; c < 3; ++c) for (int q = 0; q < cmul; ++q) for (int my = 0; my < hy; ++my) for (int mx = 0; mx < hx; ++mx) {
@@ -1204,6 +1517,7 @@
     plans->pass[f32][k] = O.slab.on ? plan_slab_pass(F, k + 1) : plan_pass(F, k + 1);
     plans->n_items[k] = F.blocks * plans->pass[f32][k].nblk;
   }
+  if (O.class_split) for (int k = 0; k < 3; ++k) plans->vm[k] = plan_vm(O, plans->pass[0][k], k + 1);
   O.plans = plans;
 }
 
@@ -1220,6 +1534,13 @@
   if (f32 && !scratch) throw Error("fdmo_apply: the fp32 transforms need the scratch array");
   double *const mid = scratch ? scratch : z_oct;
   const double *const in[3] = {g_oct, mid, mid}; double *const out[3] = {mid, mid, z_oct};
+  if (fdmo_class_split_runs(O, precision)) {
+    for (int k = 0; k < 3; ++k) {
+      OctPassVM V = O.plans->vm[k]; V.gate = gate; if (k == 1) V.gz_part = gz_part; if (k == 0) V.stop = stop;
+      launch_vm_nt(s, O.nt, V, n_items[k], in[k], out[k], ev ? ev[2 * k] : nullptr, ev ? ev[2 * k + 1] : nullptr);
+    }
+    return;
+  }
   for (int k = 0; k < 3; ++k) launch_pass_nt(s, k == 1 ? O.nt_z : O.nt, f32 ? PassVariant::OctantF32 : O.per_dir ? PassVariant::PerDirection : PassVariant::Octant, P[k], n_items[k], in[k], out[k], ev ? ev[2 * k] : nullptr, ev ? ev[2 * k + 1] : nullptr);
   stamps.dump(s);
 }
```

Result: faster. 25.45 billion (median of 6 runs) (+3.8%).
